# kemingy/rabitq

Measured on AMD Instinct MI355X. Metric: queries/sec at recall@10>=0.95, 100Mx128; HBM GB/s on popcount scan, higher is better.
Workload: dtype exact integer dot (fp6 MFMA, v_dot8_u32_u4) + f32

## Files before the change

include/rabitq_hip.h:

```cpp
#ifndef RABITQ_HIP_H
#define RABITQ_HIP_H

#include <stddef.h>
#include <stdint.h>

#ifdef __cplusplus
extern "C" {
#endif

typedef int32_t rq_status;
enum {
    RQ_OK = 0,
    RQ_ERR_INVALID = -1,
    RQ_ERR_DIM_MISMATCH = -2,
    RQ_ERR_IO = -3,
    RQ_ERR_HIP = -4,
    RQ_ERR_NO_DEVICE = -5,
    RQ_ERR_UNSUPPORTED = -6,
    RQ_ERR_EMPTY = -7,
    RQ_ERR_OOM = -8
};

typedef struct rq_index rq_index;

// ... 28 lines not shown

rq_status rq_build(const float *base, uint64_t n, uint32_t d, const float *centroids, uint32_t k,
                   const float *orthogonal, uint64_t seed, rq_index **out);
rq_status rq_build_device(const float *d_base, uint64_t n, uint32_t d, const float *d_centroids,
                          uint32_t k, const float *orthogonal_host, uint64_t seed, rq_index **out);
rq_status rq_build_from_path(const char *base_fvecs, const char *centroid_fvecs,
                             const float *orthogonal, uint64_t seed, rq_index **out);
rq_status rq_build_metric(const float *base, uint64_t n, uint32_t d, const float *centroids, uint32_t k,
                          const float *orthogonal, uint64_t seed, uint32_t metric, rq_index **out);
rq_status rq_build_device_metric(const float *d_base, uint64_t n, uint32_t d, const float *d_centroids,
                                 uint32_t k, const float *orthogonal_host, uint64_t seed, uint32_t metric, rq_index **out);
rq_status rq_build_from_path_metric(const char *base_fvecs, const char *centroid_fvecs,
                                    const float *orthogonal, uint64_t seed, uint32_t metric, rq_index **out);

typedef struct rq_builder rq_builder;
typedef struct {
    uint32_t struct_size;
    float ms_rotate, ms_assign, ms_quantize;
    uint64_t rows_assigned;
    uint64_t rows_in_hbm, rows_in_host_memory;
    uint64_t rows_exact_redo;
} rq_build_stats_t;
rq_status rq_builder_create(uint64_t n, uint32_t d, const float *d_centroids, uint32_t k, const float *orthogonal_host,
                            uint64_t seed, uint64_t max_device_base_bytes, rq_builder **out);
rq_status rq_builder_create_metric(uint64_t n, uint32_t d, const float *d_centroids, uint32_t k, const float *orthogonal_host,
                                   uint64_t seed, uint64_t max_device_base_bytes, uint32_t metric, rq_builder **out);
rq_status rq_builder_assign_chunk(rq_builder *b, const float *d_rows, uint64_t i0, uint64_t m);
rq_status rq_builder_order(rq_builder *b);
rq_status rq_builder_place_chunk(rq_builder *b, const float *d_rows, uint64_t i0, uint64_t m);
rq_status rq_builder_finish(rq_builder *b, rq_index **out);
void rq_builder_free(rq_builder *b);
rq_status rq_builder_stats(const rq_builder *b, rq_build_stats_t *out);

rq_status rq_kmeans_device(const float *d_base, uint64_t n, uint32_t d, uint32_t k, uint32_t iters,
                           uint32_t points_per_centroid, uint64_t seed, float *d_centroids_out);

rq_status rq_load_dir(const char *dir, rq_index **out);
rq_status rq_dump_dir(const rq_index *idx, const char *dir);
rq_status rq_load_json(const char *path, rq_index **out);
rq_status rq_dump_json(const rq_index *idx, const char *path);
void rq_free(rq_index *idx);

rq_status rq_from_arrays(uint32_t dim, uint64_t n, uint32_t k, const float *base,
                         const float *orthogonal, const float *centroids, const uint32_t *offsets,
                         const uint32_t *map_ids, const uint64_t *codes, const rq_factor_t *factors,
                         rq_index **out);
rq_status rq_from_arrays_metric(uint32_t dim, uint64_t n, uint32_t k, const float *base,
                                const float *orthogonal, const float *centroids, const uint32_t *offsets,
                                const uint32_t *map_ids, const uint64_t *codes, const rq_factor_t *factors,
                                uint32_t metric, rq_index **out);

rq_status rq_info(const rq_index *idx, rq_info_t *out);
enum { RQ_ARR_BASE = 0, RQ_ARR_ORTHOGONAL, RQ_ARR_CENTROIDS, RQ_ARR_OFFSETS, RQ_ARR_MAP_IDS,
       RQ_ARR_CODES, RQ_ARR_FACTORS };
rq_status rq_get_array(const rq_index *idx, int which, void *dst, uint64_t dst_bytes);
rq_status rq_get_device_ptr(const rq_index *idx, int which, const void **out_ptr, uint64_t *out_bytes);

rq_status rq_query(const rq_index *idx, const float *query, uint32_t len, uint32_t probe,
                   uint32_t topk, int heuristic_rank, float *out_dist, uint32_t *out_id,
                   uint32_t *out_n);
rq_status rq_query_batch(const rq_index *idx, const float *queries, uint32_t nq, uint32_t len,
                         uint32_t probe, uint32_t topk, int heuristic_rank, float *out_dist,
                         uint32_t *out_id, uint32_t *out_n);
rq_status rq_query_batch_device(const rq_index *idx, const float *d_queries, uint32_t nq,
                                uint32_t len, uint32_t probe, uint32_t topk, int heuristic_rank,
                                float *d_out_dist, uint32_t *d_out_id, uint32_t *d_out_n);
typedef struct rq_ticket rq_ticket;
rq_status rq_query_batch_device_begin(const rq_index *idx, const float *d_queries, uint32_t nq,
                                      uint32_t len, uint32_t probe, uint32_t topk, int heuristic_rank,
                                      float *d_out_dist, uint32_t *d_out_id, uint32_t *d_out_n,
                                      rq_ticket **out_ticket);
rq_status rq_query_batch_device_end(rq_ticket *ticket);

typedef struct rq_filter rq_filter;
rq_status rq_filter_create(const rq_index *idx, const uint32_t *allow_bits, uint64_t nbits, int bits_on_device,
                           rq_filter **out);
rq_status rq_filter_rows(const rq_filter *f, uint64_t *out_admitted);
void rq_filter_free(rq_filter *f);
rq_status rq_query_batch_filtered(const rq_index *idx, const rq_filter *filter, const float *queries, uint32_t nq,
                                  uint32_t len, uint32_t probe, uint32_t topk, int heuristic_rank, float *out_dist,
                                  uint32_t *out_id, uint32_t *out_n);
rq_status rq_query_batch_device_filtered(const rq_index *idx, const rq_filter *filter, const float *d_queries,
                                         uint32_t nq, uint32_t len, uint32_t probe, uint32_t topk, int heuristic_rank,
                                         float *d_out_dist, uint32_t *d_out_id, uint32_t *d_out_n);

typedef struct rq_range_result rq_range_result;
rq_status rq_range_search_device(const rq_index *idx, const rq_filter *filter, const float *d_queries, uint32_t nq,
                                 uint32_t len, uint32_t probe, const float *d_radius, rq_range_result **out);
rq_status rq_range_search(const rq_index *idx, const rq_filter *filter, const float *queries, uint32_t nq, uint32_t len,
                          uint32_t probe, const float *radius, rq_range_result **out);
rq_status rq_range_result_info(const rq_range_result *r, uint32_t *out_nq, uint64_t *out_total);
rq_status rq_range_result_device_ptrs(const rq_range_result *r, const uint64_t **d_lims, const float **d_dist,
                                      const uint32_t **d_id);
rq_status rq_range_result_copy(const rq_range_result *r, uint64_t *lims, float *dist, uint32_t *id);
void rq_range_result_free(rq_range_result *r);

typedef struct {
    uint32_t struct_size;
    uint32_t reserved0;
    float ms_keys, ms_assign, ms_alloc, ms_merge, ms_gather, ms_derive, ms_free, ms_total;
    uint64_t rows_before, rows_after;
    uint64_t gather_bytes;
} rq_mutate_stats_t;
rq_status rq_add(rq_index *idx, const float *rows, uint64_t m, uint32_t d, const uint32_t *ids, int rows_on_device,
                 uint32_t *out_first_id);
rq_status rq_remove(rq_index *idx, const uint32_t *id_bits, uint64_t nbits, int bits_on_device, uint64_t *out_removed);
rq_status rq_last_mutate_stats(rq_mutate_stats_t *out);
// ... 16 lines not shown
rq_status rq_partition_lists(const rq_index *idx, uint32_t world, uint32_t *out_owner, uint64_t *out_load);
rq_status rq_shard_index(const rq_index *idx, const uint32_t *owner, uint32_t rank, rq_index **out);
rq_status rq_query_batch_sharded_device(const rq_index *shard, void *nccl_comm, uint32_t world, uint32_t id_offset,
                                        const float *d_queries, uint32_t nq, uint32_t len, uint32_t probe, uint32_t topk,
                                        int heuristic_rank, float *d_out_dist, uint32_t *d_out_id, uint32_t *d_out_n);
typedef struct {
    uint32_t struct_size;
    uint32_t reserved;
    int (*all_gather)(const void *send, void *recv, size_t send_count, int dtype, void *comm, void *hip_stream);
    int (*all_reduce)(const void *send, void *recv, size_t count, int dtype, int op, void *comm, void *hip_stream);
    int (*comm_user_rank)(void *comm, int *rank);
} rq_collectives_t;
rq_status rq_set_collectives(const rq_collectives_t *collectives);

rq_status rq_metrics(rq_metrics_t *out);
rq_status rq_metrics_reset(void);

rq_status rq_rotate(const float *x, uint64_t n, uint32_t dim, const float *orthogonal, int use_mfma,
                    float *out);
rq_status rq_rotate_device(const rq_index *idx, const float *d_x, uint64_t n, float *d_out, float *out_ms);
rq_status rq_quantize_pack(const float *x_rot, uint64_t n, uint32_t dim, const float *centroids_rot,
                           uint32_t k, uint32_t *out_label, float *out_dist, uint64_t *out_codes,
                           rq_factor_t *out_factors);
rq_status rq_coarse_rank(const rq_index *idx, const float *queries, uint32_t nq, uint32_t len,
                         uint32_t probe, float *out_y, uint32_t *out_cluster, float *out_dist);
rq_status rq_query_prep(const rq_index *idx, const float *y, uint32_t nq, const uint32_t *cluster,
                        float *out_lower, float *out_delta, uint32_t *out_sum, uint64_t *out_planes);
rq_status rq_scan(const rq_index *idx, uint32_t cluster, float y_c_distance_square,
                  const uint64_t *planes, float lower_bound, float scalar_sum, float delta,
                  float *out_rough);
rq_status rq_rerank(const rq_index *idx, const float *query_padded, const uint32_t *pos, uint32_t m,
                    float *out_accurate);

typedef struct {
    uint32_t struct_size;
    uint32_t coarse_fallback_rows;
    float ms_rotate, ms_coarse, ms_select, ms_prep, ms_group, ms_scan, ms_rerank, ms_sort, ms_replay,
        ms_total;
    uint64_t scan_bytes;
    uint64_t scan_candidates;
    uint64_t rerank_candidates;
    uint32_t scan_launches;
    uint32_t retries;
    float ms_scan_matrix;
    uint32_t matrix_launches;
    uint64_t matrix_pairs;
    uint64_t matrix_subtile_steps, matrix_exact_steps;
    uint64_t rerank_shadow_rejects;
    float ms_early;
    uint32_t small_batch_passes;
    uint64_t survivor_workspace_bytes;
    uint32_t segmented_passes;
    uint32_t matrix_additive_launches;
} rq_profile_t;
rq_status rq_set_profiling(int level);
rq_status rq_set_option(const char *name, int value);
rq_status rq_last_profile(rq_profile_t *out);

#ifdef __cplusplus
}
#endif
#endif
```

rabitq_amd/_lib.py:

```python
from __future__ import annotations

import ctypes as C
import os
import subprocess

_HERE = os.path.dirname(os.path.abspath(__file__))
SO_PATH = os.environ.get("RABITQ_HIP_SO") or os.path.join(_HERE, "librabitq_hip.so")
CSRC = os.path.join(_HERE, "csrc")

RQ_OK = 0
RQ_ERR_EMPTY = -7
STATUS_NAMES = {0: "RQ_OK", -1: "RQ_ERR_INVALID", -2: "RQ_ERR_DIM_MISMATCH", -3: "RQ_ERR_IO", -4: "RQ_ERR_HIP",
                -5: "RQ_ERR_NO_DEVICE", -6: "RQ_ERR_UNSUPPORTED", -7: "RQ_ERR_EMPTY", -8: "RQ_ERR_OOM"}

EXPORTS = [
    "rq_version", "rq_abi_version", "rq_last_error", "rq_init", "rq_normalize", "rq_normalize_device", "rq_build", "rq_build_device", "rq_build_from_path",
    "rq_build_metric", "rq_build_device_metric", "rq_build_from_path_metric", "rq_builder_create_metric", "rq_from_arrays_metric", "rq_kmeans_device", "rq_builder_create", "rq_builder_assign_chunk", "rq_builder_order", "rq_builder_place_chunk", "rq_builder_finish", "rq_builder_free", "rq_builder_stats", "rq_load_dir",
    "rq_dump_dir", "rq_load_json", "rq_dump_json", "rq_free", "rq_from_arrays", "rq_info", "rq_get_array", "rq_get_device_ptr", "rq_query",
    "rq_query_batch", "rq_query_batch_device", "rq_query_batch_device_begin", "rq_query_batch_device_end", "rq_filter_create", "rq_filter_rows", "rq_filter_free", "rq_query_batch_filtered", "rq_query_batch_device_filtered", "rq_range_search", "rq_range_search_device", "rq_range_result_info", "rq_range_result_device_ptrs", "rq_range_result_copy", "rq_range_result_free", "rq_add", "rq_remove", "rq_last_mutate_stats", "rq_coarse_topk_device", "rq_merge_smallest_u64_device", "rq_query_batch_device_probed", "rq_query_batch_device_seeded", "rq_partition_lists", "rq_shard_index", "rq_query_batch_sharded_device", "rq_set_collectives", "rq_metrics", "rq_metrics_reset", "rq_rotate", "rq_rotate_device",
    "rq_quantize_pack",
    "rq_coarse_rank", "rq_query_prep", "rq_scan", "rq_rerank", "rq_set_profiling", "rq_set_option", "rq_last_profile",
]


class RabitqError(RuntimeError):
    def __init__(self, status, message):
        super().__init__(f"{STATUS_NAMES.get(status, status)}: {message}")
        self.status = status


METRIC_L2, METRIC_COSINE = 0, 1
METRICS = {"l2": METRIC_L2, "cosine": METRIC_COSINE}


def metric_id(metric) -> int:
    if isinstance(metric, str):
        if metric.lower() not in METRICS:
            raise ValueError(f"metric must be one of {sorted(METRICS)}, not {metric!r}")
        return METRICS[metric.lower()]
    return int(metric)


ABI_VERSION = 4


class _Sized(C.Structure):

    def __init__(self, *a, **kw):
        super().__init__(*a, **kw)
        self.struct_size = C.sizeof(type(self))


class Info(_Sized):
    _fields_ = [("struct_size", C.c_uint32), ("dim", C.c_uint32), ("k", C.c_uint32), ("max_list_len", C.c_uint32),
                ("n", C.c_uint64), ("n_hbm", C.c_uint64), ("split_rows", C.c_uint32), ("metric", C.c_uint32)]


class MetricsT(C.Structure):
    _fields_ = [("rough", C.c_uint64), ("precise", C.c_uint64), ("query", C.c_uint64), ("miss", C.c_uint64)]


class BuildStatsT(_Sized):
    _fields_ = [("struct_size", C.c_uint32), ("ms_rotate", C.c_float), ("ms_assign", C.c_float), ("ms_quantize", C.c_float),
                ("rows_assigned", C.c_uint64), ("rows_in_hbm", C.c_uint64), ("rows_in_host_memory", C.c_uint64),
                ("rows_exact_redo", C.c_uint64)]


class ProfileT(_Sized):
    _fields_ = [("struct_size", C.c_uint32), ("coarse_fallback_rows", C.c_uint32)] + [(n, C.c_float) for n in ("ms_rotate", "ms_coarse", "ms_select", "ms_prep", "ms_group", "ms_scan",
                                         "ms_rerank", "ms_sort", "ms_replay", "ms_total")] + [
        ("scan_bytes", C.c_uint64), ("scan_candidates", C.c_uint64), ("rerank_candidates", C.c_uint64),
        ("scan_launches", C.c_uint32), ("retries", C.c_uint32),
        ("ms_scan_matrix", C.c_float), ("matrix_launches", C.c_uint32), ("matrix_pairs", C.c_uint64),
        ("matrix_subtile_steps", C.c_uint64), ("matrix_exact_steps", C.c_uint64),
        ("rerank_shadow_rejects", C.c_uint64), ("ms_early", C.c_float), ("small_batch_passes", C.c_uint32),
        ("survivor_workspace_bytes", C.c_uint64), ("segmented_passes", C.c_uint32), ("matrix_additive_launches", C.c_uint32)]


class MutateStatsT(_Sized):
    _fields_ = [("struct_size", C.c_uint32), ("reserved0", C.c_uint32)] + [(n, C.c_float) for n in (
        "ms_keys", "ms_assign", "ms_alloc", "ms_merge", "ms_gather", "ms_derive", "ms_free", "ms_total")] + [
        ("rows_before", C.c_uint64), ("rows_after", C.c_uint64), ("gather_bytes", C.c_uint64)]


def build(force: bool = False) -> str:
    cmd = ["make", "-C", CSRC] + (["-B"] if force else [])
    subprocess.check_call(cmd, stdout=subprocess.DEVNULL)
    return SO_PATH


_lib = None


def lib():
    global _lib
    if _lib is not None:
        return _lib
    if not os.path.exists(SO_PATH):
        raise RabitqError(-5, f"{SO_PATH} not built (run `make -C rabitq_amd/csrc`); there is no CPU fallback")
    import importlib.util
    import sys
    if (not os.environ.get("RABITQ_NO_TORCH_PRELOAD") and "torch" not in sys.modules
            and importlib.util.find_spec("torch") is not None):
        try:
            import torch
        except Exception:
            pass
    L = C.CDLL(SO_PATH)
    vp, f32p, u32p, u64p = C.c_void_p, C.c_void_p, C.c_void_p, C.c_void_p
    u32, u64, i32, flt = C.c_uint32, C.c_uint64, C.c_int32, C.c_float
    pp = C.POINTER(C.c_void_p)
    sig = {
        "rq_version": (C.c_char_p, []),
        "rq_abi_version": (C.c_uint32, []),
        "rq_last_error": (C.c_char_p, []),
        "rq_init": (i32, [C.c_int]),
        "rq_build": (i32, [f32p, u64, u32, f32p, u32, f32p, u64, pp]),
        "rq_build_device": (i32, [f32p, u64, u32, f32p, u32, f32p, u64, pp]),
        "rq_build_from_path": (i32, [C.c_char_p, C.c_char_p, f32p, u64, pp]),
        "rq_normalize": (i32, [f32p, u64, u32, f32p]),
        "rq_normalize_device": (i32, [f32p, u64, u32, f32p]),
        "rq_build_metric": (i32, [f32p, u64, u32, f32p, u32, f32p, u64, u32, pp]),
        "rq_build_device_metric": (i32, [f32p, u64, u32, f32p, u32, f32p, u64, u32, pp]),
        "rq_build_from_path_metric": (i32, [C.c_char_p, C.c_char_p, f32p, u64, u32, pp]),
        "rq_builder_create_metric": (i32, [u64, u32, f32p, u32, f32p, u64, u64, u32, pp]),
        "rq_from_arrays_metric": (i32, [u32, u64, u32, f32p, f32p, f32p, u32p, u32p, u64p, vp, u32, pp]),
        "rq_kmeans_device": (i32, [f32p, u64, u32, u32, u32, u32, u64, f32p]),
        "rq_builder_create": (i32, [u64, u32, f32p, u32, f32p, u64, u64, pp]),
        "rq_builder_assign_chunk": (i32, [vp, f32p, u64, u64]),
# ... 69 lines not shown
```

rabitq_amd/csrc/host_build.h:

```cpp
#pragma once
#define RQ_SHADOW_MIN_ROWS 1ull
static std::atomic<int> g_rerank_shadow{2};
static rq_status derive_shadow_rows(rq_index *idx);
static rq_status finish_index(rq_index *idx) {
    idx->W = idx->dim / 64;
    RQC(idx->cent_t.alloc((size_t)idx->dim * idx->k));
    RQC(ensure_kernel_attributes());
    if (idx->k)
        transpose_kernel<<<dim3(ceil_div(idx->dim, 32), ceil_div(idx->k, 32)), dim3(32, 8)>>>(
            idx->centroids.p, idx->cent_t.p, idx->k, idx->dim);
    DevBuf<uint32_t> mx;
    RQC(mx.alloc(2));
    const uint32_t mx_init[2] = {0u, 0xFFFFFFFFu};
    HIPC(hipMemcpy(mx.p, mx_init, 8, hipMemcpyHostToDevice));
    if (idx->k) max_list_len_kernel<<<ceil_div(idx->k, 256), 256>>>(idx->offsets.p, idx->k, mx.p);
    uint32_t mx_out[2];
    HIPC(hipMemcpy(mx_out, mx.p, 8, hipMemcpyDeviceToHost));
    idx->max_list_len = mx_out[0];
    idx->min_list_len = idx->k ? mx_out[1] : 0;
    {
        DevBuf<uint32_t> st4;
        RQC(st4.alloc(4));
        HIPC(hipMemset(st4.p, 0, 16));
        if (idx->n)
            factor_stats_kernel<<<(uint32_t)std::min<uint64_t>(ceil_div(idx->n, 256), 4096), 256>>>(idx->factors.p, idx->n, st4.p);
        HIPC(hipMemcpy(&idx->fstats, st4.p, 16, hipMemcpyDeviceToHost));
    }
    idx->cent_norm_max = INFINITY;
    if (idx->k) {
        const uint64_t cells = (uint64_t)idx->k * idx->dim;
        DevBuf<uint32_t> mxb;
        RQC(mxb.alloc(1));
        HIPC(hipMemset(mxb.p, 0, 4));
        RQC(idx->cent_bf.alloc(cells));
        RQC(idx->cent_sqnorm.alloc(idx->k));
        to_bf16_kernel<<<ceil_div(cells, 2048), 256>>>(idx->centroids.p, cells, idx->cent_bf.p);
        row_sqnorm_kernel<<<ceil_div(idx->k, 256), 256>>>(idx->centroids.p, idx->k, idx->dim, idx->cent_sqnorm.p, mxb.p);
        float m2 = 0.0f;
        HIPC(hipMemcpy(&m2, mxb.p, 4, hipMemcpyDeviceToHost));
        idx->cent_norm_max = std::isfinite(m2) && m2 < 1.0e30f ? std::sqrt(m2) * 1.000001f : INFINITY;
    }
    if (idx->k) {
        RQC(idx->list_uref.alloc(idx->k));
        list_uref_kernel<<<idx->k, 256>>>(idx->factors.p, idx->offsets.p, idx->list_uref.p);
    }
    HIPC(hipDeviceSynchronize());
    HIPC(hipGetLastError());
    RQC(derive_shadow_rows(idx));
    idx->h_offsets.resize((size_t)idx->k + 1);
    HIPC(hipMemcpy(idx->h_offsets.data(), idx->offsets.p, ((size_t)idx->k + 1) * 4, hipMemcpyDeviceToHost));
    idx->nonempty_lists = 0;
    for (uint32_t c = 0; c < idx->k; ++c) idx->nonempty_lists += idx->h_offsets[c + 1] > idx->h_offsets[c] ? 1u : 0u;
    {
        size_t free_b = 0, total_b = 0;
        HIPC(hipMemGetInfo(&free_b, &total_b));
        idx->pass_budget = std::min<uint64_t>(std::max<uint64_t>(free_b / 3, 4ull << 30), 96ull << 30);
    }
    return RQ_OK;
}

static rq_status derive_shadow_rows(rq_index *idx) {
    idx->base_h.release();
    idx->base_q8.release();
    idx->list_q8.release();
    int kind = g_rerank_shadow.load();
    if (kind == 2 && idx->dim > 4096) kind = 1;
    if (!kind || idx->base_host != nullptr || idx->split_rows || idx->n < RQ_SHADOW_MIN_ROWS) return RQ_OK;
    const uint64_t total = idx->n * idx->dim, bytes = total * (kind == 2 ? 1 : 2);
    size_t free_b = 0, total_b = 0;
    HIPC(hipMemGetInfo(&free_b, &total_b));
    if (free_b < bytes + (48ull << 30) && bytes > (1ull << 30)) return RQ_OK;
    if (kind == 2) {
        if (idx->base_q8.alloc(total) != RQ_OK || idx->list_q8.alloc(std::max<uint32_t>(idx->k, 1)) != RQ_OK) {
            (void)hipGetLastError();
            idx->base_q8.release();
            idx->list_q8.release();
            return RQ_OK;
        }
        std::vector<uint32_t> off((size_t)idx->k + 1);
        HIPC(hipMemcpy(off.data(), idx->offsets.p, off.size() * 4, hipMemcpyDeviceToHost));
        uint32_t longest = 0;
        for (uint32_t c = 0; c < idx->k; ++c) longest = std::max(longest, off[c + 1] - off[c]);
        q8_range_kernel<<<idx->k, 256>>>(idx->base.p, idx->offsets.p, idx->dim, idx->list_q8.p);
        if (longest)
            for (uint32_t c0 = 0; c0 < idx->k; c0 += 32768)
                q8_encode_kernel<<<dim3(ceil_div(longest, 256u), std::min(32768u, idx->k - c0)), 256>>>(
                    idx->base.p, idx->offsets.p + c0, idx->dim, idx->list_q8.p + c0, idx->base_q8.p);
        HIPC(hipDeviceSynchronize());
        HIPC(hipGetLastError());
        return RQ_OK;
    }
    if (idx->base_h.alloc(total) != RQ_OK) {
        (void)hipGetLastError();
        return RQ_OK;
    }
    half_rows_kernel<<<(uint32_t)std::min<uint64_t>(ceil_div(total, 2048), 1u << 20), 256>>>(idx->base.p, total, idx->base_h.p);
    HIPC(hipDeviceSynchronize());
    HIPC(hipGetLastError());
    return RQ_OK;
}

static void gen_orthogonal(uint32_t dim, uint64_t seed, std::vector<float> &out) {
    std::mt19937_64 rng(seed);
    std::normal_distribution<double> nd(0.0, 1.0);
    const size_t D = dim;
    std::vector<double> A(D * D), Q(D * D, 0.0), v(D);
    for (auto &a : A) a = nd(rng);
    std::vector<std::vector<double>> vs;
    vs.reserve(D);
    for (size_t j = 0; j < D; ++j) {
        double norm = 0;
        for (size_t i = j; i < D; ++i) norm += A[i * D + j] * A[i * D + j];
        norm = std::sqrt(norm);
        std::vector<double> h(D, 0.0);
        double alpha = A[j * D + j] > 0 ? -norm : norm;
        for (size_t i = j; i < D; ++i) h[i] = A[i * D + j];
        h[j] -= alpha;
        double hn = 0;
        for (size_t i = j; i < D; ++i) hn += h[i] * h[i];
        if (hn > 0) {
            for (size_t c = j; c < D; ++c) {
                double dot = 0;
                for (size_t i = j; i < D; ++i) dot += h[i] * A[i * D + c];
                dot = 2 * dot / hn;
                for (size_t i = j; i < D; ++i) A[i * D + c] -= dot * h[i];
            }
        }
        vs.push_back(std::move(h));
    }
    for (size_t i = 0; i < D; ++i) Q[i * D + i] = 1.0;
    for (size_t jj = D; jj-- > 0;) {
        const auto &h = vs[jj];
        double hn = 0;
        for (size_t i = jj; i < D; ++i) hn += h[i] * h[i];
        if (hn == 0) continue;
        for (size_t c = 0; c < D; ++c) {
            double dot = 0;
            for (size_t i = jj; i < D; ++i) dot += h[i] * Q[i * D + c];
            dot = 2 * dot / hn;
            for (size_t i = jj; i < D; ++i) Q[i * D + c] -= dot * h[i];
// ... 670 lines not shown
```

rabitq_amd/csrc/host_mutate.h:

```cpp
#pragma once

static thread_local rq_mutate_stats_t g_mutate_stats;
struct PhaseClock {
    std::chrono::steady_clock::time_point t = std::chrono::steady_clock::now();
    float lap() {
        const auto now = std::chrono::steady_clock::now();
        const float ms = std::chrono::duration<float, std::milli>(now - t).count();
        t = now;
        return ms;
    }
};

static rq_status ensure_row_keys(rq_index *idx) {
    if (idx->row_key_valid) return RQ_OK;
    PhaseClock clk;
    const uint64_t n = idx->n;
    const uint32_t dim = idx->dim;
    DevBuf<uint32_t> rk;
    RQC(rk.alloc(n));
    if (n) {
        const uint64_t chunk = std::min<uint64_t>(n, std::max<uint64_t>(64, (256ull << 20) / ((uint64_t)dim * 4)));
        DevBuf<float> xrot;
        RQC(xrot.alloc(chunk * dim));
        for (uint64_t r0 = 0; r0 < n; r0 += chunk) {
// ... 104 lines not shown
    RQC(nx->base.alloc(n * dim));
    RQC(nx->codes.alloc(n * W));
    RQC(nx->factors.alloc(n));
    RQC(nx->map_ids.alloc(n));
    RQC(nx->row_key.alloc(n));
    DevBuf<uint32_t> src_of_dst, empty_off;
    DevBuf<unsigned int> holes;
    RQC(src_of_dst.alloc(n));
    RQC(holes.alloc(1));
    HIPC(hipMemset(holes.p, 0, 4));
    HIPC(hipMemset(src_of_dst.p, 0xFF, n * 4));
    HIPC(hipMemcpy(nx->P.p, idx->P.p, (size_t)dim * dim * 4, hipMemcpyDeviceToDevice));
    HIPC(hipMemcpy(nx->centroids.p, idx->centroids.p, (size_t)k * dim * 4, hipMemcpyDeviceToDevice));
    HIPC(hipMemcpy(nx->offsets.p, h_out.data(), ((size_t)k + 1) * 4, hipMemcpyHostToDevice));
    const uint32_t *new_off = nullptr;
    if (nr) {
        new_off = nr->off.p;
    } else {
        RQC(empty_off.alloc((size_t)k + 1));
        HIPC(hipMemset(empty_off.p, 0, ((size_t)k + 1) * 4));
        new_off = empty_off.p;
    }
    HIPC(hipDeviceSynchronize());
    st.ms_alloc = clk.lap();
    const unsigned long long *nkeys = nr ? nr->keys.p : nullptr;
    const uint32_t *nids = nr && nr->ids.p ? nr->ids.p : nullptr, *nsrc = nr && nr->src.p ? nr->src.p : nullptr;
    const uint32_t id0 = nr ? nr->id0 : 0u;
    if (k)
        mutate_merge_kernel<<<k, 256>>>(idx->offsets.p, idx->row_key.p, idx->map_ids.p, drop_bits, new_off, nkeys, nids, id0,
                                        nx->offsets.p, (uint32_t)n_old, src_of_dst.p);
    HIPC(hipDeviceSynchronize());
    st.ms_merge = clk.lap();
    if (n)
        mutate_gather_kernel<<<(uint32_t)std::min<uint64_t>(ceil_div(n, 4), 1u << 20), 256>>>(
            src_of_dst.p, n, (uint32_t)n_old, nr ? (uint32_t)nr->m : 0u, dim, W, idx->base.p, idx->codes.p, idx->factors.p, idx->map_ids.p, idx->row_key.p,
            nkeys, nids, id0, nsrc, nr ? nr->rows : nullptr, nr ? nr->d : dim, nr ? nr->b->codes_tmp.p : nullptr,
            nr ? nr->b->factors_tmp.p : nullptr, nx->base.p, nx->codes.p, nx->factors.p, nx->map_ids.p, nx->row_key.p, holes.p);
    HIPC(hipDeviceSynchronize());
    HIPC(hipGetLastError());
    st.ms_gather = clk.lap();
    st.gather_bytes = 2 * n * ((uint64_t)dim * 4 + (uint64_t)W * 8 + 16 + 4 + 4) + n * 4;
    unsigned int h_holes = 0;
    HIPC(hipMemcpy(&h_holes, holes.p, 4, hipMemcpyDeviceToHost));
    if (h_holes)
        return fail(RQ_ERR_HIP, "internal: the merge left " + std::to_string(h_holes) + " rows of the new layout unset");
    src_of_dst.release();
    if (nr) nr->b.reset();
    RQC(finish_index(nx.get()));
    nx->row_key_valid = true;
    st.ms_derive = clk.lap();

    swap_buf(idx->base, nx->base), swap_buf(idx->P, nx->P), swap_buf(idx->centroids, nx->centroids), swap_buf(idx->cent_t, nx->cent_t);
    swap_buf(idx->base_h, nx->base_h), swap_buf(idx->base_q8, nx->base_q8), swap_buf(idx->list_q8, nx->list_q8);
    swap_buf(idx->offsets, nx->offsets), swap_buf(idx->map_ids, nx->map_ids), swap_buf(idx->codes, nx->codes);
    swap_buf(idx->factors, nx->factors), swap_buf(idx->list_uref, nx->list_uref), swap_buf(idx->cent_bf, nx->cent_bf);
    swap_buf(idx->cent_sqnorm, nx->cent_sqnorm), swap_buf(idx->row_key, nx->row_key);
    idx->n = nx->n, idx->n_dev = nx->n_dev, idx->max_list_len = nx->max_list_len, idx->min_list_len = nx->min_list_len;
    idx->cent_norm_max = nx->cent_norm_max, idx->nonempty_lists = nx->nonempty_lists, idx->fstats = nx->fstats;
    idx->pass_budget = nx->pass_budget;
    idx->h_offsets.swap(nx->h_offsets);
    idx->row_key_valid = true;
    {
        std::lock_guard<std::mutex> g(idx->tt_mu);
        idx->tile_tables.clear();
    }
    {
        std::lock_guard<std::mutex> g(idx->ws_mu);
        idx->ws_pool.clear();
    }
    ++idx->generation;
    nx.reset();
    HIPC(hipDeviceSynchronize());
    st.ms_free = clk.lap();
    if (!idx->base_q8.p && !idx->base_h.p) (void)derive_shadow_rows(idx);
    size_t free_b = 0, total_b = 0;
    if (hipMemGetInfo(&free_b, &total_b) == hipSuccess)
        idx->pass_budget = std::min<uint64_t>(std::max<uint64_t>(free_b / 3, 4ull << 30), 96ull << 30);
    (void)hipGetLastError();
    st.ms_derive += clk.lap();
    return RQ_OK;
}

static rq_status scan_ids(const rq_index *idx, const uint32_t *sorted, uint64_t m, uint64_t *top, uint64_t *hits) {
    DevBuf<unsigned long long> out;
    RQC(out.alloc(2));
    HIPC(hipMemset(out.p, 0, 16));
    if (idx->n)
        id_scan_kernel<<<(uint32_t)std::min<uint64_t>(ceil_div(idx->n, 256), 4096), 256>>>(idx->map_ids.p, idx->n, sorted, (uint32_t)m, out.p);
    unsigned long long h[2];
    HIPC(hipMemcpy(h, out.p, 16, hipMemcpyDeviceToHost));
    *top = h[0], *hits = h[1];
    return RQ_OK;
}

static void mutate_stats_begin(const rq_index *idx) {
    g_mutate_stats = rq_mutate_stats_t{};
    g_mutate_stats.struct_size = sizeof(rq_mutate_stats_t);
    g_mutate_stats.rows_before = g_mutate_stats.rows_after = idx ? idx->n : 0;
}

static rq_status index_add(rq_index *idx, const float *rows, uint64_t m, uint32_t d, const uint32_t *ids, int rows_on_device,
                           uint32_t *out_first_id) {
    RQC(ensure_device());
    RQC(ensure_kernel_attributes());
    mutate_stats_begin(idx);
    RQC(mutate_refusals(idx));
// ... 100 lines not shown
```

rabitq_amd/csrc/host_plan.h:

```cpp
#pragma once
struct QueryParams {
    uint32_t nq, len, probe, topk;
    bool heuristic;
    uint32_t cap, hcap;
    const float *thr_init = nullptr;
    bool seg_final = false;
    bool ext_lists = false;
    const rq_filter *filter = nullptr;
    bool range = false;
};

#define RQ_DEFAULT_CAP 4096u
#define RQ_MAX_CAP_HINT 32768u
#define RQ_MAX_NQ_PER_PASS 65536u
#define RQ_MAX_PROBE 16384u

#define RQ_PREP_SHAPES(X) X(128, 16, 2, 16, 2) X(64, 16, 1, 16, 4) X(256, 32, 2, 8, 2) X(512, 32, 4, 8, 1) X(768, 32, 6, 8, 1) X(1024, 32, 8, 8, 1)

struct StagePlan {
    uint32_t s_lo, s_hi;
    uint64_t span, est_pairs;
    bool matrix;
    bool cluster_major;
    bool ranked;
    bool additive;
    bool arena_stage;
    bool placed;
    bool want_table;
    uint32_t slot_hi, stage_pairs;
    uint32_t dense_cells;
    uint32_t tile, tiles_per_group;
};

struct PassPlan {
    uint32_t nprobe, npairs;
    uint32_t dbg;
    bool small;
    uint32_t sb_nstages, sb_lo[RQ_SB_MAX_STAGES], sb_hi[RQ_SB_MAX_STAGES], sb_final_lo;
    bool sb_whole, sb_fill_final;
    bool will_list;
    bool placed;
    bool fin_additive;
    bool write_qn, write_q6;
    uint32_t qn_slots;
    uint32_t prep_lp, prep_r, prep_ppb, prep_pp;
    uint32_t mid_blocks;
    uint32_t nstages;
    StagePlan st[RQ_MAX_STAGES];
};

static void plan_stages(const rq_index *idx, uint32_t nq, uint32_t nprobe, uint64_t first_hi, uint64_t growth, uint64_t settle_cap, PassPlan &pl) {
    pl.nstages = 0;
    const uint64_t total_max = std::min<uint64_t>((uint64_t)nprobe * idx->max_list_len, idx->n);
    uint64_t lo = 0, hi = first_hi;
    const uint64_t avg = std::max<uint64_t>(1, idx->n / std::max<uint32_t>(idx->nonempty_lists, 1));
    uint64_t settle = std::min(settle_cap, std::max<uint64_t>(avg, std::min<uint64_t>(idx->max_list_len, 16 * avg)));
    if (rq_large_batch(nq)) settle = std::max<uint64_t>(1, settle * (uint64_t)g_stage_settle_pct.load() / 100);
    while (lo < total_max) {
        const bool last = hi >= total_max || lo >= settle || pl.nstages + 1 == RQ_MAX_STAGES;
        pl.st[pl.nstages++] = StagePlan{(uint32_t)lo, last ? 0xFFFFFFFFu : (uint32_t)hi};
        if (last) break;
        lo = hi;
        hi = std::min<uint64_t>(hi * growth, 0xFFFFFFF0ull);
        if (lo < 2 * avg && 2 * hi > 2 * avg) hi = 2 * avg;
        if (lo < settle && hi > settle) hi = settle;
    }
}

static void plan_pass(const rq_index *idx, const QueryParams &qp, bool has_row_map, bool ext_lists, PassPlan &pl) {
    const uint32_t dim = idx->dim, k = idx->k, W = idx->W;
    const uint32_t nq = qp.nq, nprobe = std::min(qp.probe, k), topk = qp.topk;
    const uint32_t npairs = nq * nprobe;
    const rq_filter *filt = qp.filter;
    const bool large = rq_large_batch(nq), fused = scan_is_fused(W);
    pl = PassPlan{};
    pl.nprobe = nprobe, pl.npairs = npairs;
    const uint32_t min_len = filt ? 0u : idx->min_list_len;
    const int impl = g_scan_impl.load();
    pl.dbg = (uint32_t)g_scan_dbg.load();
    const int gate_opt = g_scan_gate.load(), rank_opt = g_group_rank.load(), tt_opt = g_scan_tile_table.load(), gopt = g_stage_growth.load();
    const bool dense_opt = g_dense_dir.load() != 0, additive_loose = idx->additive_loose.load() != 0;
    const uint64_t settle_pct = (uint64_t)g_stage_settle_pct.load();
    const uint64_t avg_len = std::max<uint64_t>(1, idx->n / std::max<uint32_t>(idx->nonempty_lists, 1));
    const uint64_t total_max = std::min<uint64_t>((uint64_t)nprobe * idx->max_list_len, idx->n);
    const bool one_stage = qp.range || (qp.thr_init != nullptr && !has_row_map);

    const bool sb_w = W == 1 || W == 2 || W == 4 || W == 8 || W == 12 || W == 16;
    pl.small = g_small_batch.load() == 0 && nq <= RQ_SB_MAX_NQ && !ext_lists && !has_row_map && !qp.thr_init && !filt && sb_w &&
               k <= RQ_SB_MAX_K && nprobe <= 64 && topk <= RQ_SB_MAX_TOPK && qp.cap <= 4 * RQ_DEFAULT_CAP;
    if (pl.small) {
        plan_stages(idx, nq, nprobe, 16ull * std::max<uint32_t>(topk, 1), gopt >= 2 ? (uint64_t)gopt : 8, (uint64_t)std::max(1, g_sb_span.load()), pl);
        if (pl.nstages > RQ_SB_MAX_STAGES) pl.small = false;
    }
    if (pl.small) {
        const bool whole = pl.sb_whole = pl.nstages == 0 || (total_max - pl.st[pl.nstages - 1].s_lo) * (uint64_t)(dim / 8 + 16) <= (1ull << 20);
        pl.sb_nstages = whole ? pl.nstages : pl.nstages - 1;
        for (uint32_t i = 0; i < pl.sb_nstages; ++i) pl.sb_lo[i] = pl.st[i].s_lo, pl.sb_hi[i] = pl.st[i].s_hi;
        const StagePlan fin = whole ? StagePlan{} : pl.st[pl.nstages - 1];
        pl.sb_fill_final = !whole && !(npairs >= k / 2 && npairs > 64);
        pl.sb_final_lo = fin.s_lo;
        pl.nstages = 0;
        if (!whole) pl.st[pl.nstages++] = fin;
    } else if (one_stage) {
        pl.nstages = 1;
        pl.st[0] = StagePlan{0u, 0xFFFFFFFFu};
    } else {
        const uint64_t growth = gopt >= 2 ? (uint64_t)gopt : (nq >= 32768 ? 8 : 16);
        plan_stages(idx, nq, nprobe, (uint64_t)std::max<uint32_t>(topk, 1) * (large ? growth : 1), growth, ~0ull, pl);
    }

    for (uint32_t i = 0; i < pl.nstages; ++i) {
        StagePlan &s = pl.st[i];
        s.span = (uint64_t)std::min<uint64_t>(s.s_hi, (uint64_t)nprobe * idx->max_list_len) - s.s_lo;
        s.est_pairs = (uint64_t)nq * std::min<uint64_t>(nprobe, s.span / avg_len + 2);
        s.matrix = scan_has_mfma(W) && impl != 1 &&
                   (impl == 2 || (s.est_pairs >= 8ull * k && (s.s_lo >= avg_len * settle_pct / 100 || one_stage)));
        s.cluster_major = s.matrix || (s.est_pairs >= k / (pl.small ? 2u : (uint32_t)g_cluster_major_div.load()) && s.est_pairs > 64);
        s.arena_stage = qp.seg_final && s.span > qp.cap && fused && large;
        s.additive = s.matrix && !s.arena_stage && !filt && scan_has_additive(W) && idx->list_uref.p != nullptr && gate_opt != 1 &&
                     (gate_opt == 2 || !additive_loose);
        s.slot_hi = nprobe;
        if (s.cluster_major && min_len > 0 && !ext_lists && s.s_hi != 0xFFFFFFFFu)
            s.slot_hi = (uint32_t)std::min<uint64_t>(nprobe, (uint64_t)(s.s_hi - 1) / min_len + 1);
        s.stage_pairs = nq * s.slot_hi;
        s.ranked = s.cluster_major && k <= 32768 &&
                   (rank_opt == 2 || (rank_opt == 1 && s.stage_pairs >= 16 * RQ_RANK_ITEMS && s.stage_pairs / RQ_RANK_ITEMS >= k / 256));
        s.tile = s.matrix ? scan_mfma_tile(W, s.arena_stage, s.additive) : scan_tile(W);
        s.tiles_per_group = ceil_div(std::min<uint64_t>(idx->max_list_len, s.s_hi), s.tile);
        const uint64_t grid_blocks = (uint64_t)k * s.tiles_per_group, real_tiles = idx->n / s.tile + k;
        s.want_table = s.cluster_major && fused && s.s_hi >= idx->max_list_len && (tt_opt == 2 || (tt_opt == 1 && grid_blocks > 4 * real_tiles));
        if (large && !s.matrix && fused && dense_opt && s.s_hi != 0xFFFFFFFFu && !(qp.seg_final && s.span > qp.cap)) {
            const uint64_t cells = (uint64_t)((s.s_hi - 1) >> 6) - (s.s_lo >> 6) + 2ull * s.slot_hi + 2;
// ... 40 lines not shown
```

rabitq_amd/csrc/host_query.h:

```cpp
#pragma once
static rq_status ws_prepare(const rq_index *idx, Workspace &ws, const QueryParams &qp) {
    const uint32_t nprobe = std::min(qp.probe, idx->k);
    const uint64_t nq = qp.nq, npairs = nq * nprobe;
    if (!ws.stream) HIPC(hipStreamCreateWithFlags(&ws.stream, hipStreamNonBlocking));
    if (!ws.h_totals) HIPC(hipHostMalloc((void **)&ws.h_totals, 16 * sizeof(unsigned long long)));
    RQC(ws.qpad.ensure(nq * idx->dim));
    RQC(ws.y.ensure(nq * idx->dim));
    if (!qp.ext_lists) RQC(ws.dist.ensure(nq * idx->k));
    RQC(ws.probe_dist.ensure(npairs));
    RQC(ws.probe_cluster.ensure(npairs));
    RQC(ws.scal.ensure(npairs));
    if (!scan_is_fused(idx->W)) RQC(ws.planes.ensure(npairs * 4 * idx->W));
    RQC(ws.qnib.ensure(npairs * 8 * idx->W));
    RQC(ws.qf6.ensure(npairs * 12 * idx->W));
    RQC(ws.rough_cnt.ensure(nq));
    RQC(ws.totals.ensure(16));
    RQC(ws.stat.ensure(256));
    RQC(ws.recs.ensure((npairs + 32ull * idx->k + 32) * (12ull * idx->W + 2 + RQ_REC_TAIL)));
    RQC(ws.grp_cnt.ensure(idx->k + 4));
    RQC(ws.grp_start.ensure(idx->k + 1));
    RQC(ws.q_hist.ensure(idx->k + 2));
    RQC(ws.q_start.ensure(idx->k + 2));
    RQC(ws.q_order.ensure(nq));
    RQC(ws.thr.ensure(nq));
    RQC(ws.surv.ensure(nq * qp.cap));
    RQC(ws.runs.ensure(nq * qp.cap));
    ws.use_runs_tmp = qp.cap > RQ_DEFAULT_CAP || qp.seg_final || hints_of(idx, qp.filter).big_dirs.load() > 0;
    if (ws.use_runs_tmp) RQC(ws.runs_tmp.ensure(nq * qp.cap));
    RQC(ws.surv_cnt.ensure(nq));
    RQC(ws.heap_len.ensure(nq));
    RQC(ws.heap_key.ensure(nq * qp.topk));
    RQC(ws.heap_id.ensure(nq * qp.topk));
    RQC(ws.precise.ensure(nq));
    RQC(ws.need.ensure(nq));
    RQC(ws.ovf.ensure(nq));
    RQC(ws.q_cap.ensure(nq));
    RQC(ws.q_base.ensure(nq));
    RQC(ws.nsurv.ensure(nq));
    RQC(ws.nshadow.ensure(nq));
    RQC(ws.recent.ensure(nq));
    RQC(ws.win_count.ensure(nq));
    RQC(ws.arr_len.ensure(nq));
    RQC(ws.row_map.ensure(nq));
    RQC(ws.big_list.ensure(nq + 3));
    if (qp.heuristic) RQC(ws.arr.ensure(nq * qp.hcap));
    return RQ_OK;
}

struct PassResult {
    uint64_t rough = 0, precise = 0, overflowed = 0, max_need = 0;
};

static rq_status finish_pass(const rq_index *idx, Workspace &ws, PassResult *res, rq_profile_t *prof_acc) {
    Prof &pf = ws.prof;
    const uint32_t nq = ws.pend.nq, dim = idx->dim;
    HIPC(hipStreamSynchronize(ws.stream));
    HIPC(hipGetLastError());
    res->rough = ws.h_totals[0];
    res->precise = ws.h_totals[1];
    res->overflowed = ws.h_totals[2];
    res->max_need = ws.h_totals[4];
    if (rq_large_batch(nq) && !ws.pend.range) hints_of(idx, ws.pend.filter).big_dirs.store((uint32_t)ws.h_totals[7]);
    if (ws.pend.additive && !ws.pend.range && ws.h_totals[8] >= 4096 && ws.h_totals[9] * 32 > ws.h_totals[8])
        const_cast<rq_index *>(idx)->additive_loose.store(1);
    if (prof_acc) prof_acc->matrix_subtile_steps += ws.h_totals[8], prof_acc->matrix_exact_steps += ws.h_totals[9];
    if (prof_acc) prof_acc->coarse_fallback_rows += (uint32_t)std::min<unsigned long long>(ws.h_totals[10], 0xFFFFFFFFull);
    if (pf.on && prof_acc) {
        float ms[PF_N] = {0};
        pf.collect(ms);
        prof_acc->ms_rotate += ms[PF_ROTATE], prof_acc->ms_coarse += ms[PF_COARSE];
        prof_acc->ms_select += ms[PF_SELECT], prof_acc->ms_prep += ms[PF_PREP], prof_acc->ms_group += ms[PF_GROUP];
        prof_acc->ms_scan += ms[PF_SCAN] + ms[PF_SCAN_MATRIX], prof_acc->ms_scan_matrix += ms[PF_SCAN_MATRIX];
        prof_acc->ms_rerank += ms[PF_RERANK], prof_acc->ms_sort += ms[PF_SORT];
        if (ws.pend.n_matrix_ranges) {
            std::vector<unsigned long long> len(nq);
            HIPC(hipMemcpy(len.data(), ws.pend.filter ? ws.stream_len.p : ws.rough_cnt.p, (size_t)nq * 8, hipMemcpyDeviceToHost));
            for (uint32_t i = 0; i < ws.pend.n_matrix_ranges; ++i) {
                const StreamRange r = ws.pend.matrix_ranges[i];
                for (uint32_t b = 0; b < nq; ++b)
                    prof_acc->matrix_pairs += std::min<unsigned long long>(len[b], r.s_hi) - std::min<unsigned long long>(len[b], r.s_lo);
            }
        }
        prof_acc->ms_replay += ms[PF_REPLAY], prof_acc->ms_total += ms[PF_TOTAL], prof_acc->ms_early += ms[PF_EARLY];
    }
    if (prof_acc) {
        const uint64_t slots = std::max<uint64_t>((uint64_t)nq * ws.pend.cap, ws.pend.seg_slots);
        prof_acc->survivor_workspace_bytes = std::max<uint64_t>(prof_acc->survivor_workspace_bytes,
            ws.pend.seg_slots ? (ws.surv.count + ws.runs.count + ws.runs_tmp.count + ws.arena_recs.count + ws.arena_runs.count) * 16ull
                              : slots * (ws.use_runs_tmp ? 48ull : 32ull));
        prof_acc->segmented_passes += ws.pend.seg_slots ? 1u : 0u;
        prof_acc->scan_candidates += res->rough;
        prof_acc->scan_bytes += res->rough * (uint64_t)(dim / 8 + 16);
        prof_acc->rerank_candidates += ws.h_totals[3];
        prof_acc->rerank_shadow_rejects += ws.h_totals[5];
        if (g_scan_dbg.load() & 256) {
            unsigned long long ht[12];
            HIPC(hipMemcpy(ht, ws.stat.p + 128, sizeof ht, hipMemcpyDeviceToHost));
            if (ht[3])
                fprintf(stderr, "[rabitq_hip] scan_mfma exact path (wave 0 of every block): %.0f cycles per block inside it (of which flushes %.0f), "
                        "%.1f flagged registers, %.1f with survivors and %.2f flushes per block\n", (double)ht[5] / ht[3], (double)ht[6] / ht[3],
                        (double)ht[9] / ht[3], (double)ht[7] / ht[3], (double)ht[8] / ht[3]);
            if (ht[3])
                fprintf(stderr, "[rabitq_hip] scan_mfma timing: %llu blocks, %.1f tiles/block; per block cycles: start-up %.0f, "
                        "tile-loop waits %.0f, tile bodies %.0f (per tile: wait %.0f, body %.0f)\n", ht[3], (double)ht[4] / ht[3],
                        (double)ht[0] / ht[3], (double)ht[1] / ht[3], (double)ht[2] / ht[3], (double)ht[1] / std::max(1ull, ht[4]),
                        (double)ht[2] / std::max(1ull, ht[4]));
        }
        if ((g_scan_dbg.load() & 4096) && nq <= RQ_SB_MAX_NQ) {
            unsigned long long hs[32];
            HIPC(hipMemcpy(hs, ws.stat.p, sizeof hs, hipMemcpyDeviceToHost));
            std::string line = "[rabitq_hip] sb_query_kernel phases (us since entry):";
            for (unsigned long long i = 1; i < std::min<unsigned long long>(hs[0], 30); ++i) line += " " + std::to_string((hs[1 + i] - hs[1]) / 100.0).substr(0, 6);
            fprintf(stderr, "%s\n", line.c_str());
        }
    }
    return RQ_OK;
}

struct StageRun {
    const StagePlan &s;
    uint32_t no;
    ScanArgs a{};
    ScanPtrs sp{};
    QSeg seg{};
    bool runs_in_tmp = false;
};
struct Pass {
    const rq_index *idx;
    Workspace &ws;
    const QueryParams &qp;
    const PassPlan &pl;
    Prof &pf;
    hipStream_t st;
    const uint32_t dim, k, W, nq, topk, nprobe, npairs;
    const float *d_q;
    const uint32_t *d_row_map, *ext_cluster;
    const float *ext_dist;
    float *d_out_dist;
    uint32_t *d_out_id, *d_out_n;
    rq_profile_t *prof_acc;
    const float *qpad;
    const uint32_t *probe_cluster;
    const float *probe_dist;
    ReplayState rs;
    const uint32_t *rerank_order = nullptr;
    uint32_t nlive = 0;
    bool sb_results_done = false;
// ... 342 lines not shown
            if (s.dense_cells) {
                pf.begin(PF_SORT);
                clear_dir_kernel<<<ceil_div((uint64_t)qp.nq * s.dense_cells, 256), 256, 0, st>>>(ws.runs.p, qp.nq, r.seg, s.dense_cells);
                pf.end();
            }
            stage_launch_scan(r);
        }
        if (s.matrix) pend.matrix_stages++;
        if (prof_acc && s.additive) prof_acc->matrix_additive_launches++;
        if (prof_acc) prof_acc->scan_launches++;
        if (prof_acc && s.matrix) {
            prof_acc->matrix_launches++;
            pend.matrix_ranges[pend.n_matrix_ranges++] = {s.s_lo, s.s_hi};
        }
        return RQ_OK;
    }

    void stage_finish_small(StageRun &r) {
        const QSeg &seg = r.seg;
        pf.begin(PF_RERANK);
        const uint32_t fin_threads = nq <= 16 ? 1024u : 256u;
        uint32_t flags = qp.cap > RQ_DEFAULT_CAP && nprobe <= 1024 ? 1u : 0u;
        if (flags) {
            sort_runs_kernel<<<nq, 64, 0, st>>>(ws.runs.p, ws.surv_cnt.p, seg, ws.big_list.p, ws.big_list.p + nq, RQ_SORT_LDS_RECS, nullptr);
            sort_runs_mid_kernel<<<std::min(nq, 256u), 256, RQ_SORT_MID_LDS_WORDS * 8, st>>>(ws.runs.p, ws.use_runs_tmp ? ws.runs_tmp.p : nullptr, ws.surv_cnt.p,
                                                                                          seg, ws.big_list.p, ws.big_list.p + nq, nprobe, 0u,
                                                                                          RQ_SORT_MID_LDS_WORDS);
        }
        if (pl.small && !qp.heuristic) {
            if (nq <= 32) {
                accurate_kernel<<<dim3(std::max(1u, std::min(16u, 256u / nq)), nq), 256, (size_t)dim * sizeof(float), st>>>(
                    ws.surv.p, ws.surv_cnt.p, seg, idx->view(), qpad, dim, nullptr, probe_cluster, nprobe);
                flags |= 2u;
            }
            auto finish = topk < 64 ? sb_finish_kernel<true> : sb_finish_kernel<false>;
            finish<<<nq, fin_threads, (size_t)dim * sizeof(float) + (2 * RQ_SBF_RUNS + RQ_SBF_RECS) * 16, st>>>(
                ws.surv.p, ws.runs.p, ws.surv_cnt.p, seg, idx->view(), qpad, dim, topk, rs, probe_cluster, nprobe, flags,
                idx->map_ids.p, d_out_dist, d_out_id, d_out_n, ws.rough_cnt.p, ws.totals.p);
            sb_results_done = true;
        } else {
            auto finish = qp.heuristic ? stage_finish_kernel<true> : stage_finish_kernel<false>;
            finish<<<nq, fin_threads, (size_t)dim * sizeof(float), st>>>(ws.surv.p, ws.runs.p, ws.surv_cnt.p, seg, idx->view(), qpad, dim, topk, rs,
                                                                         probe_cluster, nprobe, flags);
        }
        pf.end();
    }

    void stage_finish_large(StageRun &r) {
        const uint32_t dense_cells = r.s.dense_cells;
        const QSeg &seg = r.seg;
        pf.begin(PF_RERANK);
        const uint32_t gx = std::max(1u, std::min(16u, 4096u / std::max(nq, 1u)));
        const bool prefilter = (r.no > 0 || qp.thr_init) && !(pl.dbg & 512);
        if (idx->base_q8.p && prefilter)
            accurate_filtered8_kernel<<<dim3(gx, nq), 256, (size_t)dim * sizeof(float) + (nprobe <= RQ_ACC8_LDS_PROBES ? (size_t)nprobe * 16 : 0), st>>>(
                ws.surv.p, ws.surv_cnt.p, seg, idx->base.p, idx->base_q8.p, idx->list_q8.p, qpad, dim, rerank_order, ws.thr.p,
                probe_cluster, nprobe, ws.nshadow.p, k);
        else if (idx->base_h.p && prefilter)
            accurate_filtered_kernel<<<dim3(gx, nq), 256, (size_t)dim * sizeof(float), st>>>(
                ws.surv.p, ws.surv_cnt.p, seg, idx->base.p, idx->base_h.p, qpad, dim, rerank_order, ws.thr.p,
                ws.nshadow.p);
        else if (idx->split_rows && prefilter)
            accurate_split_kernel<<<dim3(gx, nq), 256, (size_t)dim * sizeof(float) + (nprobe <= RQ_ACC8_LDS_PROBES ? (size_t)nprobe * 16 : 0), st>>>(
                ws.surv.p, ws.surv_cnt.p, seg, idx->view(), qpad, dim, rerank_order, ws.thr.p, probe_cluster, nprobe, ws.nshadow.p);
        else
            accurate_kernel<<<dim3(gx, nq), 256, (size_t)dim * sizeof(float), st>>>(ws.surv.p, ws.surv_cnt.p, seg, idx->view(), qpad, dim,
                                                                                    rerank_order, probe_cluster, nprobe);
        if (qp.range)
            range_count_kernel<<<ceil_div(nq, 4), 256, 0, st>>>(ws.surv.p, ws.surv_cnt.p, qp.cap, ws.thr.p, nq, ws.range_hits.p, ws.need.p,
                                                                ws.ovf.p, ws.precise.p, ws.nsurv.p);
        pf.end();
        if (qp.range) return;
        if (!dense_cells) {
            pf.begin(PF_SORT);
            sort_runs_kernel<<<nq, 64, 0, st>>>(ws.runs.p, ws.surv_cnt.p, seg, ws.big_list.p, ws.big_list.p + nq, 512u,
                                                r.runs_in_tmp ? ws.runs_tmp.p : nullptr);
            sort_runs_mid_kernel<<<pl.mid_blocks, 256, RQ_SORT_MID_LDS_WORDS * 8, st>>>(ws.runs.p, (ws.use_runs_tmp || r.runs_in_tmp) ? ws.runs_tmp.p : nullptr,
                                                                                       ws.surv_cnt.p, seg, ws.big_list.p, ws.big_list.p + nq, nprobe,
                                                                                       r.runs_in_tmp ? 1u : 0u, RQ_SORT_MID_LDS_WORDS);
            pf.end();
        }
        pf.begin(PF_REPLAY);
        if (qp.heuristic)
            replay_kernel<true><<<nq, 64, 16, st>>>(ws.surv.p, ws.runs.p, ws.surv_cnt.p, seg, topk, rs, dense_cells);
        else if (topk < 64)
            replay_kernel<false, true><<<nq, 64, 16, st>>>(ws.surv.p, ws.runs.p, ws.surv_cnt.p, seg, topk, rs, dense_cells);
        else
            replay_kernel<false><<<nq, 64, (size_t)topk * 8, st>>>(ws.surv.p, ws.runs.p, ws.surv_cnt.p, seg, topk, rs, dense_cells);
        pf.end();
    }

    rq_status results(size_t total_span) {
        pf.begin(PF_REPLAY);
        if (!sb_results_done) {
            if (qp.heuristic && !qp.range) {
                sort_survivors_kernel<<<nq, 256, 0, st>>>(ws.arr.p, ws.arr_len.p, qp.hcap);
                finalize_heuristic_kernel<<<ceil_div((uint64_t)nq * topk, 256), 256, 0, st>>>(rs, nq, topk, d_row_map, idx->map_ids.p,
                                                                                               d_out_dist, d_out_id, d_out_n);
            } else if (!qp.range) {
                finalize_heap_kernel<<<ceil_div((uint64_t)nq * topk, 256), 256, 0, st>>>(rs, nq, topk, d_row_map, idx->map_ids.p, d_out_dist,
                                                                                          d_out_id, d_out_n);
            }
            metrics_sum_kernel<<<std::min(256u, ceil_div(nq, 256)), 256, 0, st>>>(
                ws.rough_cnt.p, ws.precise.p, ws.need.p, qp.heuristic ? ws.arr_len.p : nullptr, ws.nsurv.p, ws.nshadow.p, nq, ws.ovf.p, qp.hcap,
                ws.totals.p);
        }
        pf.end();
        if (pf.on) (void)hipEventRecord(pf.spans[total_span].b, st);
        HIPC(hipMemcpyAsync(ws.h_totals, ws.totals.p, 7 * sizeof(unsigned long long), hipMemcpyDeviceToHost, st));
        ws.h_totals[7] = 0, ws.h_totals[8] = 0, ws.h_totals[9] = 0, ws.h_totals[10] = 0;
        if (pend.prefiltered) HIPC(hipMemcpyAsync(ws.h_totals + 10, ws.totals.p + 12, 8, hipMemcpyDeviceToHost, st));
        if (pend.matrix_stages) {
            stat_fold_kernel<<<1, 64, 0, st>>>(ws.stat.p, ws.stat.p + 200);
            HIPC(hipMemcpyAsync(ws.h_totals + 8, ws.stat.p + 200, 16, hipMemcpyDeviceToHost, st));
        }
        if (rq_large_batch(nq))
            HIPC(hipMemcpyAsync(ws.h_totals + 7, ws.big_list.p + nq + 2, 4, hipMemcpyDeviceToHost, st));
        ws.pend = pend;
        return RQ_OK;
    }
};

static rq_status run_pass(const rq_index *idx, Workspace &ws, const float *d_q, const QueryParams &qp,
                          const uint32_t *d_row_map, float *d_out_dist, uint32_t *d_out_id, uint32_t *d_out_n,
                          PassResult *res, rq_profile_t *prof_acc, const uint32_t *ext_cluster = nullptr,
                          const float *ext_dist = nullptr, bool defer = false) {
    PassPlan pl;
    plan_pass(idx, qp, d_row_map != nullptr, ext_cluster != nullptr, pl);
    Pass c{idx, ws, qp, pl, ws.prof, ws.stream, idx->dim, idx->k, idx->W, qp.nq, qp.topk, pl.nprobe, pl.npairs, d_q, d_row_map, ext_cluster, ext_dist,
           d_out_dist, d_out_id, d_out_n, prof_acc, d_q, ws.probe_cluster.p, ws.probe_dist.p};
    c.rs.thr = ws.thr.p, c.rs.heap_len = ws.heap_len.p, c.rs.heap_key = ws.heap_key.p, c.rs.heap_id = ws.heap_id.p;
    c.rs.precise = ws.precise.p, c.rs.need = ws.need.p, c.rs.nsurv = ws.nsurv.p, c.rs.nshadow = ws.nshadow.p, c.rs.recent_max = ws.recent.p, c.rs.win_count = ws.win_count.p;
    c.rs.arr_len = ws.arr_len.p, c.rs.arr = ws.arr.p, c.rs.hcap = qp.hcap, c.rs.ovf = ws.ovf.p;
    c.pend.nq = qp.nq, c.pend.cap = qp.cap, c.pend.filter = qp.filter, c.pend.range = qp.range;
    Prof &pf = ws.prof;
    pf.reset(g_profiling.load(), ws.stream);
    pf.begin(PF_TOTAL);
    const size_t total_span = pf.spans.size() ? pf.spans.size() - 1 : 0;
    if (pl.small) {
        RQC(c.small_front());
    } else {
        RQC(c.rotate_coarse());
        if (pl.placed) RQC(c.place_final());
        pf.begin(PF_PREP);
        RQC(c.quantise());
        RQC(c.orders_state());
        pf.end();
    }
    for (uint32_t i = 0; i < pl.nstages; ++i) {
        StageRun r{pl.st[i], i};
        RQC(c.stage_group_fill(r));
        RQC(c.stage_scan(r));
        if (!qp.range && !rq_large_batch(qp.nq) && qp.cap <= 4 * RQ_DEFAULT_CAP) c.stage_finish_small(r);
        else c.stage_finish_large(r);
    }
    RQC(c.results(total_span));
    if (defer) return RQ_OK;
    return finish_pass(idx, ws, res, prof_acc);
}

static rq_status validate_call(const rq_index *idx, bool args_null, uint32_t len, uint32_t probe, uint32_t topk, const rq_filter *filter) {
    RQC(ensure_device());
    RQC(ensure_kernel_attributes());
    if (!idx || args_null) return fail(RQ_ERR_INVALID, "null argument");
    if (idx->dim != (len + 63) / 64 * 64)
        return fail(RQ_ERR_DIM_MISMATCH, "query length " + std::to_string(len) + " does not pad to index dim " +
                                             std::to_string(idx->dim));
    if (probe == 0 || idx->k == 0) return fail(RQ_ERR_INVALID, "probe == 0 (the reference panics at rabitq.rs:295)");
    if (topk == 0 || topk > RQ_MAX_TOPK) return fail(RQ_ERR_UNSUPPORTED, "topk must be in [1, 2048]");
    if (std::min(probe, idx->k) > RQ_MAX_PROBE) return fail(RQ_ERR_UNSUPPORTED, "probe > 16384 not supported");
    if (idx->dim > 4096) return fail(RQ_ERR_UNSUPPORTED, "dim > 4096 not supported");
    if (filter && filter->idx != idx) return fail(RQ_ERR_INVALID, "the filter was made for another index");
    if (filter && filter->generation != idx->generation)
        return fail(RQ_ERR_INVALID, "the filter was made before the index was last mutated (rq_add / rq_remove): make it again");
    return RQ_OK;
}
static rq_status validate_query(const rq_index *idx, const float *d_q, uint32_t len, uint32_t probe, uint32_t topk,
                                const float *d_out_dist, const uint32_t *d_out_id, const uint32_t *d_out_n, const rq_filter *filter = nullptr) {
    return validate_call(idx, !d_q || !d_out_dist || !d_out_id || !d_out_n, len, probe, topk, filter);
}

static uint32_t pass_capacity(const rq_index *idx, uint32_t remaining, bool seeded, bool *seg, const rq_filter *filter = nullptr) {
    const uint32_t hint = hints_of(idx, filter).cap.load();
    const int opt = g_seg_opt.load();
    *seg = !seeded && rq_large_batch(remaining) && scan_is_fused(idx->W) && (opt >= 2 || (opt == 1 && hint > RQ_DEFAULT_CAP));
// ... 309 lines not shown
```

rabitq_amd/csrc/host_shard.h:

```cpp
#pragma once
rq_status rq_partition_lists(const rq_index *idx, uint32_t world, uint32_t *out_owner, uint64_t *out_load) {
    if (!idx || !out_owner || world == 0) return fail(RQ_ERR_INVALID, "bad partition arguments");
    std::vector<uint32_t> off((size_t)idx->k + 1);
    RQC(rq_get_array(idx, RQ_ARR_OFFSETS, off.data(), off.size() * 4));
    std::vector<uint32_t> order(idx->k);
    for (uint32_t c = 0; c < idx->k; ++c) order[c] = c;
    std::stable_sort(order.begin(), order.end(),
                     [&](uint32_t a, uint32_t b) { return off[a + 1] - off[a] > off[b + 1] - off[b]; });
    typedef std::pair<uint64_t, uint32_t> LS;
    std::priority_queue<LS, std::vector<LS>, std::greater<LS>> heap;
    for (uint32_t r = 0; r < world; ++r) heap.push({0, r});
    for (uint32_t c : order) {
        LS t = heap.top();
        heap.pop();
        out_owner[c] = t.second;
        t.first += off[c + 1] - off[c];
        heap.push(t);
    }
    if (out_load) {
        for (uint32_t r = 0; r < world; ++r) out_load[r] = 0;
        for (uint32_t c = 0; c < idx->k; ++c) out_load[out_owner[c]] += off[c + 1] - off[c];
    }
    return RQ_OK;
}
// ... 37 lines not shown
}

struct RcclApi {
    int (*all_gather)(const void *, void *, size_t, int, void *, hipStream_t) = nullptr;
    int (*all_reduce)(const void *, void *, size_t, int, int, void *, hipStream_t) = nullptr;
    int (*user_rank)(void *, int *) = nullptr;
    const char *(*error_string)(int) = nullptr;
    std::string err;
};
static RcclApi g_custom_coll;
static std::atomic<bool> g_use_custom_coll{false};
static RcclApi *rccl_api() {
    if (g_use_custom_coll.load()) return &g_custom_coll;
    static RcclApi api;
    static std::once_flag once;
    std::call_once(once, [] {
        void *h = nullptr;
        const char *env = getenv("RABITQ_RCCL_LIB");
        if (env && *env) h = dlopen(env, RTLD_NOW | RTLD_GLOBAL);
        void *sym = h ? dlsym(h, "ncclAllGather") : dlsym(RTLD_DEFAULT, "ncclAllGather");
        if (!sym && !h) {
            for (const char *name : {"librccl.so.1", "librccl.so"}) {
                h = dlopen(name, RTLD_NOW | RTLD_GLOBAL);
                if (h) break;
            }
            sym = h ? dlsym(h, "ncclAllGather") : nullptr;
        }
        if (!sym) {
            api.err = "RCCL not found (ncclAllGather): set RABITQ_RCCL_LIB to the librccl.so the communicator came from";
            return;
        }
        auto find = [&](const char *name) { return h ? dlsym(h, name) : dlsym(RTLD_DEFAULT, name); };
        api.all_gather = reinterpret_cast<decltype(api.all_gather)>(sym);
        api.all_reduce = reinterpret_cast<decltype(api.all_reduce)>(find("ncclAllReduce"));
        api.user_rank = reinterpret_cast<decltype(api.user_rank)>(find("ncclCommUserRank"));
        api.error_string = reinterpret_cast<decltype(api.error_string)>(find("ncclGetErrorString"));
    });
    return &api;
}
#define RQ_NCCL_INT32 2
#define RQ_NCCL_UINT64 5
#define RQ_NCCL_FLOAT32 7
#define RQ_NCCL_MAX 2
#define RQ_NCCL_MIN 3

static void profile_add(rq_profile_t &acc, const rq_profile_t &x) {
    acc.ms_rotate += x.ms_rotate, acc.ms_coarse += x.ms_coarse, acc.ms_select += x.ms_select, acc.ms_prep += x.ms_prep;
    acc.ms_group += x.ms_group, acc.ms_scan += x.ms_scan, acc.ms_rerank += x.ms_rerank, acc.ms_sort += x.ms_sort;
    acc.ms_replay += x.ms_replay, acc.ms_total += x.ms_total, acc.scan_bytes += x.scan_bytes;
    acc.scan_candidates += x.scan_candidates, acc.rerank_candidates += x.rerank_candidates, acc.scan_launches += x.scan_launches;
    acc.retries += x.retries, acc.ms_scan_matrix += x.ms_scan_matrix, acc.matrix_launches += x.matrix_launches;
    acc.matrix_pairs += x.matrix_pairs, acc.matrix_subtile_steps += x.matrix_subtile_steps;
    acc.matrix_exact_steps += x.matrix_exact_steps, acc.rerank_shadow_rejects += x.rerank_shadow_rejects;
    acc.ms_early += x.ms_early, acc.small_batch_passes += x.small_batch_passes;
    acc.survivor_workspace_bytes = std::max(acc.survivor_workspace_bytes, x.survivor_workspace_bytes), acc.segmented_passes += x.segmented_passes;
    acc.matrix_additive_launches += x.matrix_additive_launches;
    acc.coarse_fallback_rows += x.coarse_fallback_rows;
}

__global__ void pack_probe_keys_kernel(const uint32_t *__restrict__ pc, const float *__restrict__ pd, uint64_t cells,
                                       unsigned long long *__restrict__ keys) {
    const uint64_t i = (uint64_t)blockIdx.x * blockDim.x + threadIdx.x;
    if (i < cells) keys[i] = ((unsigned long long)__builtin_bit_cast(uint32_t, pd[i]) << 32) | pc[i];
}
__global__ void unpack_probe_keys_kernel(const unsigned long long *__restrict__ keys, uint32_t nq, uint32_t npb,
                                         uint32_t *__restrict__ pc, float *__restrict__ pd, uint32_t *__restrict__ pc_a,
                                         float *__restrict__ pd_a, uint32_t *__restrict__ pc_b, float *__restrict__ pd_b) {
    const uint64_t i = (uint64_t)blockIdx.x * blockDim.x + threadIdx.x;
    if (i >= (uint64_t)nq * npb) return;
    const uint32_t b = (uint32_t)(i / npb), c = (uint32_t)(i - (uint64_t)b * npb);
    const unsigned long long key = keys[i];
    const uint32_t id = (uint32_t)key;
    const float dv = __builtin_bit_cast(float, (uint32_t)(key >> 32));
    pc[i] = id, pd[i] = dv;
    if (!pc_a) return;
    if (c == 0) pc_a[b] = id, pd_a[b] = dv;
    else pc_b[(uint64_t)b * (npb - 1) + c - 1] = id, pd_b[(uint64_t)b * (npb - 1) + c - 1] = dv;
}
__global__ void gather_status_kernel(const unsigned long long *__restrict__ gathered, uint32_t world, uint64_t rank_stride,
                                     uint64_t at, uint32_t *__restrict__ flag) {
    uint32_t bad = 0;
    for (uint32_t w = 0; w < world; ++w) bad |= gathered[(uint64_t)w * rank_stride + at] != 0ull ? (w + 1u) : 0u;
    *flag = bad;
}

static rq_status sharded_step(rq_index *mi, void *nccl_comm, uint32_t world, uint32_t id_offset, const float *d_queries,
                              uint32_t nq, uint32_t len, uint32_t probe, uint32_t topk, bool heuristic, float *d_out_dist,
                              uint32_t *d_out_id, uint32_t *d_out_n, bool shared) {
    RcclApi *api = nccl_comm ? rccl_api() : nullptr;
    if (api && (!api->all_gather || !api->all_reduce))
        return fail(RQ_ERR_UNSUPPORTED, api->err.empty() ? "ncclAllGather / ncclAllReduce not found" : api->err);
    if (api && world > 1 && !api->user_rank) return fail(RQ_ERR_UNSUPPORTED, "ncclCommUserRank not found");
    auto nccl_fail = [&](const char *what, int rc) {
        return fail(RQ_ERR_HIP, std::string(what) + ": " + (api && api->error_string ? api->error_string(rc) : "error " + std::to_string(rc)));
    };
    const uint32_t npb = std::min(probe, std::max(mi->k, 1u));
    const uint32_t width = shared ? 2 * topk : topk;
    Workspace *ws = ws_acquire(mi);
    WsLease rel(mi, ws);
    if (!ws->stream) HIPC(hipStreamCreateWithFlags(&ws->stream, hipStreamNonBlocking));
    hipStream_t st = ws->stream;
    RQC(ws->sh_flag.ensure(8));
    const uint64_t cells = (uint64_t)nq * topk, pcells = (uint64_t)nq * npb;
    const uint64_t out_stride = (uint64_t)nq * width + 1;
    int my_rank = 0;
    rq_status err = validate_query(mi, d_queries, len, probe, topk, d_out_dist, d_out_id, d_out_n);
// ... 164 lines not shown
```

rabitq_amd/csrc/host_state.h:

```cpp
#pragma once
static thread_local std::string g_err;
static rq_status fail(rq_status s, const std::string &msg) {
    g_err = msg;
    return s;
}
#define HIPC(expr)                                                                                   \
    do {                                                                                             \
        hipError_t _e = (expr);                                                                      \
        if (_e != hipSuccess)                                                                        \
            return fail(_e == hipErrorOutOfMemory ? RQ_ERR_OOM : RQ_ERR_HIP,                         \
                        std::string(#expr) + ": " + hipGetErrorString(_e));                          \
    } while (0)
#define RQC(expr)                        \
    do {                                 \
        rq_status _s = (expr);           \
        if (_s != RQ_OK) return _s;      \
    } while (0)

static rq_status ensure_device() {
    int count = 0;
    hipError_t e = hipGetDeviceCount(&count);
    if (e != hipSuccess || count == 0)
        return fail(RQ_ERR_NO_DEVICE, "no HIP device visible (librabitq_hip has no CPU fallback)");
    return RQ_OK;
// ... 111 lines not shown
    void reset(int level, hipStream_t st) {
        on = level != 0;
        light = level == 2;
        stream = st;
        spans.clear();
        used = 0;
        open = false;
        last_b = nullptr;
        failed = false;
    }
    void collect(float *ms ) {
        if (failed) return;
        for (auto &s : spans) {
            float t = 0;
            (void)hipEventElapsedTime(&t, s.a, s.b);
            ms[s.cat] += t;
        }
    }
    ~Prof() {
        for (auto e : pool) (void)hipEventDestroy(e);
    }
};

struct StreamRange {
    uint32_t s_lo, s_hi;
};
#define RQ_MAX_STAGES 40
struct PendingPass {
    uint64_t seg_slots = 0;
    uint32_t cap = 0;
    uint32_t nq = 0;
    StreamRange matrix_ranges[RQ_MAX_STAGES];
    uint32_t n_matrix_ranges = 0;
    const struct rq_filter *filter = nullptr;
    bool additive = false;
    uint32_t matrix_stages = 0;
    bool prefiltered = false;
    bool range = false;
};
struct Workspace {
    hipStream_t stream = nullptr;
    bool busy = false;
    PendingPass pend;
    DevBuf<float> qpad, y, dist, probe_dist, thr, recent;
    DevBuf<float> qnorm;
    DevBuf<float> retry_q, retry_pd, retry_pc;
    DevBuf<uint32_t> retry_rows;
    DevBuf<uint32_t> q_hist, q_start, q_order;
    DevBuf<uint32_t> live_list;
    DevBuf<uint32_t> coarse_redo;
    DevBuf<uint32_t> pair_rank, rank_base;
    DevBuf<uint32_t> img_final, pair_begin, fin_rank, fin_rank_base, fin_grp_cnt, fin_grp_start;
    DevBuf<uint32_t> probe_cluster, recs, grp_cnt, grp_start, heap_len, heap_id, precise, need,
        nsurv, nshadow, win_count, arr_len, row_map, big_list;
    DevBuf<int32_t> heap_key;
    DevBuf<PairScalars> scal;
    DevBuf<uint64_t> planes;
    DevBuf<uint32_t> qnib;
    DevBuf<uint32_t> qf6;
    DevBuf<unsigned long long> rough_cnt, totals, surv_cnt, stat;
    DevBuf<unsigned long long> stream_len;
    DevBuf<float4> grp_vref;
    DevBuf<SurvRec> surv, arr;
    DevBuf<RunRec> runs, runs_tmp;
    bool use_runs_tmp = false;
    bool arena_failed = false;
    DevBuf<float> sh_dist;
    DevBuf<uint32_t> sh_id, sh_n;
    DevBuf<unsigned long long> sh_packed, sh_gathered, sh_merged;
    DevBuf<uint32_t> range_hits;
    DevBuf<uint32_t> range_lists;
    DevBuf<unsigned long long> range_counters;
    DevBuf<uint32_t> ovf, q_cap;
    DevBuf<unsigned long long> q_base;
    DevBuf<SurvRec> arena_recs;
    DevBuf<RunRec> arena_runs;
    DevBuf<uint2> arena_places;
    DevBuf<unsigned long long> arena_cur;
    DevBuf<unsigned int> arena_fail;
    DevBuf<ScanExtra> scan_extra;
    DevBuf<uint32_t> sh_flag;
    DevBuf<uint32_t> sh_pc, sh_id_b, sh_n_b;
    DevBuf<float> sh_pd, sh_thr, sh_dist_b;
    unsigned long long *h_totals = nullptr;
    Prof prof;
    ~Workspace() {
        if (h_totals) (void)hipHostFree(h_totals);
        if (stream) (void)hipStreamDestroy(stream);
    }
};

struct rq_index {
    uint32_t dim = 0, k = 0, W = 0, max_list_len = 0;
    uint32_t min_list_len = 0;
    uint64_t n = 0;
    uint32_t metric = RQ_METRIC_L2;
    uint64_t n_dev = 0;
    float *base_host = nullptr;
    float *base_host_dev = nullptr;
    DevBuf<ListTier> list_tier;
    std::vector<ListTier> h_list_tier;
    bool split_rows = false;
    BaseView view() const { return BaseView{base.p, base_host_dev, list_tier.p, k, split_rows ? 1u : 0u}; }
    ~rq_index() {
        if (base_host) (void)hipHostFree(base_host);
    }
    DevBuf<float> base, P, centroids, cent_t;
    DevBuf<_Float16> base_h;
    DevBuf<uint8_t> base_q8;
    DevBuf<float4> list_q8;
    DevBuf<uint32_t> offsets, map_ids;
    DevBuf<uint64_t> codes;
    DevBuf<float4> factors;
    DevBuf<float4> list_uref;
    DevBuf<uint16_t> cent_bf;
    DevBuf<float> cent_sqnorm;
    float cent_norm_max = INFINITY;
    uint32_t nonempty_lists = 0;
    std::atomic<int> additive_loose{0};
    std::mutex ws_mu;
    std::vector<std::unique_ptr<Workspace>> ws_pool;
    FactorStats fstats{0, 0, 0, 0};
    std::atomic<uint32_t> cap_hint{0};
    std::atomic<uint64_t> arena_hint{0};
    std::atomic<uint32_t> big_dirs_hint{0};
    std::atomic<uint32_t> range_cap_hint{0};
    uint64_t pass_budget = 24ull << 30;
    std::vector<uint32_t> h_offsets;
    std::mutex tt_mu;
    std::map<uint32_t, std::unique_ptr<DevBuf<uint4>>> tile_tables;
    DevBuf<uint32_t> row_key;
    bool row_key_valid = false;
    bool row_order_ok = true;
    bool is_shard = false;
    uint64_t generation = 0;
    std::atomic<int> open_tickets{0};
};

struct rq_filter {
    const rq_index *idx = nullptr;
    uint64_t generation = 0;
    DevBuf<uint32_t> pos_bits;
    DevBuf<uint32_t> sub_off;
    DevBuf<ScanExtra> extra;
    uint64_t rows = 0;
    std::atomic<uint32_t> cap_hint{0};
    std::atomic<uint64_t> arena_hint{0};
    std::atomic<uint32_t> big_dirs_hint{0};
};
struct PassHints {
    std::atomic<uint32_t> &cap;
    std::atomic<uint64_t> &arena;
    std::atomic<uint32_t> &big_dirs;
};
static PassHints hints_of(const rq_index *idx, const rq_filter *f) {
    if (f) {
        rq_filter *m = const_cast<rq_filter *>(f);
        return PassHints{m->cap_hint, m->arena_hint, m->big_dirs_hint};
    }
    rq_index *m = const_cast<rq_index *>(idx);
    return PassHints{m->cap_hint, m->arena_hint, m->big_dirs_hint};
}

// ... 246 lines not shown
    const uint32_t gchunk = std::max(1u, maxb / tchunk);
    for (uint32_t t0 = 0; t0 < a.tiles_per_group; t0 += tchunk)
        for (uint32_t g0 = 0; g0 < a.ngroups; g0 += gchunk) {
            ScanArgs c = a;
            c.tile_base = t0, c.group_base = g0;
            c.tiles_per_group = std::min(tchunk, a.tiles_per_group - t0);
            c.ngroups = std::min(gchunk, a.ngroups - g0);
            launch(c, dim3(c.ngroups * c.tiles_per_group));
        }
}

#define SCAN_ARGS p.codes, p.factors, p.offsets, p.grp_start, p.recs, p.surv, p.runs, p.surv_cnt, p.tile_table, a
template <bool ARENA, bool FILT>
static void launch_scan_t(const ScanPtrs &p, const ScanArgs &args, uint32_t W, hipStream_t st) {
    launch_scan_chunks(args, [&](const ScanArgs &a, dim3 g) {
        const dim3 b(256);
#define RQ_SCAN_K(WW, CPL)                                                                        \
    do {                                                                                          \
        if constexpr (FILT) scan_kernel<WW, CPL, ARENA, true><<<g, b, 0, st>>>(SCAN_ARGS);         \
        else scan_kernel<WW, CPL, ARENA><<<g, b, 0, st>>>(SCAN_ARGS);                             \
    } while (0)
        switch (W) {
            case 1: RQ_SCAN_K(1, 2); break;
            case 2: RQ_SCAN_K(2, 2); break;
            case 3: RQ_SCAN_K(3, 2); break;
            case 4: RQ_SCAN_K(4, 2); break;
            case 6: RQ_SCAN_K(6, 2); break;
            case 8: RQ_SCAN_K(8, 2); break;
            case 12: RQ_SCAN_K(12, 1); break;
            case 16: RQ_SCAN_K(16, 1); break;
            default:
                if constexpr (!ARENA && FILT) scan_generic_filtered_kernel<<<g, b, 0, st>>>(SCAN_ARGS, W);
                else if constexpr (!ARENA) scan_generic_kernel<<<g, b, 0, st>>>(SCAN_ARGS, W);
                break;
        }
#undef RQ_SCAN_K
    });
}
static void launch_scan(const ScanPtrs &p, const ScanArgs &args, uint32_t W, hipStream_t st) {
    if (p.filtered) {
        if (p.arena) launch_scan_t<true, true>(p, args, W, st);
        else launch_scan_t<false, true>(p, args, W, st);
    } else if (p.arena) launch_scan_t<true, false>(p, args, W, st);
    else launch_scan_t<false, false>(p, args, W, st);
}
static std::atomic<int> g_scan_impl{0};
static std::atomic<int> g_scan_gate{0};
static std::atomic<int> g_stage_growth{0};
static std::atomic<int> g_large_from{256};
static bool rq_large_batch(uint32_t nq) { return nq >= (uint32_t)g_large_from.load(); }
static std::atomic<int> g_cluster_major_div{32};
static std::atomic<int> g_stage_settle_pct{100};
static std::atomic<int> g_scan_tile_table{1};
static std::atomic<int> g_prep_placement{1};
static std::atomic<int> g_group_rank{1};
static std::atomic<int> g_shared_thr{1};
static std::atomic<int> g_sb_span{2560};
static std::atomic<int> g_seg_opt{1};
static std::atomic<int> g_pass_overlap{1};
static std::atomic<int> g_small_batch{0};
static std::atomic<int> g_dense_dir{1};

static bool scan_has_mfma(uint32_t W) {
    switch (W) {
        case 1: case 2: case 3: case 4: case 6: case 8: case 12: case 16: return true;
        default: return false;
    }
}
static uint32_t scan_mfma_nt(uint32_t W, bool additive = false) { return W == 2 ? (additive ? RQ_ADD_NT2 : RQ_NT_W2) : (W == 12 ? RQ_NT_W12 : (W >= 4 ? 2 : 4)); }
static uint32_t scan_mfma_nw(uint32_t W, bool arena) { return W == 2 && !arena ? 8u : 4u; }
static uint32_t scan_mfma_tile(uint32_t W, bool arena, bool additive = false) { return 32 * scan_mfma_nw(W, arena) * scan_mfma_nt(W, additive && !arena); }
static size_t scan_mfma_ring_bytes(uint32_t W, bool arena = false) {
    (void)arena;
    const uint64_t slots = W <= 2 ? 4ull : (W >= 16 ? 5ull : 3ull);
    return slots * (32 * (12 * W + 2) + RQ_REC_TAIL * 32) * 4;
}
template <int W, int NT, bool ARENA, bool ADD = false, bool FILT = false>
static void launch_scan_mfma_t(const ScanPtrs &p, const ScanArgs &a, dim3 g, hipStream_t st) {
    scan_mfma_kernel<W, NT, ARENA, ADD, FILT><<<g, dim3(64 * scan_mfma_waves<W, ARENA>()), scan_mfma_ring_bytes(W, ARENA), st>>>(p.codes, p.factors, p.offsets, p.grp_start, p.grp_cnt,
                                                                                    p.recs, p.surv, p.runs, p.surv_cnt, p.stat, p.tile_table, p.list_uref, p.grp_vref, a);
}
static bool scan_has_additive(uint32_t W) { return W == 1 || W == 2; }
static void launch_scan_mfma_add(const ScanPtrs &p, const ScanArgs &args, uint32_t W, hipStream_t st) {
    launch_scan_chunks(args, [&](const ScanArgs &a, dim3 g) {
        switch (W) {
            case 1: launch_scan_mfma_t<1, 4, false, true>(p, a, g, st); break;
            case 2: launch_scan_mfma_t<2, RQ_ADD_NT2, false, true>(p, a, g, st); break;
            default: break;
        }
    });
}
template <bool ARENA, bool FILT = false>
static void launch_scan_mfma_a(const ScanPtrs &p, const ScanArgs &args, uint32_t W, hipStream_t st) {
    launch_scan_chunks(args, [&](const ScanArgs &a, dim3 g) {
        switch (W) {
            case 1: launch_scan_mfma_t<1, 4, ARENA, false, FILT>(p, a, g, st); break;
            case 2: launch_scan_mfma_t<2, RQ_NT_W2, ARENA, false, FILT>(p, a, g, st); break;
            case 3: launch_scan_mfma_t<3, 4, ARENA, false, FILT>(p, a, g, st); break;
            case 4: launch_scan_mfma_t<4, 2, ARENA, false, FILT>(p, a, g, st); break;
            case 6: launch_scan_mfma_t<6, 2, ARENA, false, FILT>(p, a, g, st); break;
            case 8: launch_scan_mfma_t<8, 2, ARENA, false, FILT>(p, a, g, st); break;
            case 12: launch_scan_mfma_t<12, RQ_NT_W12, ARENA, false, FILT>(p, a, g, st); break;
            case 16: launch_scan_mfma_t<16, 2, ARENA, false, FILT>(p, a, g, st); break;
            default: break;
        }
    });
// ... 111 lines not shown
```

rabitq_amd/csrc/kernels_query.h:

```cpp
#pragma once
#ifndef RQ_COLLECT_UNROLL
#define RQ_COLLECT_UNROLL 8
#endif
#include "common.h"
#include "kernels_scan_common.h"

#pragma clang fp contract(off)

__global__ void pad_rows_kernel(const float *__restrict__ in, float *__restrict__ out, uint64_t n,
                                uint32_t len, uint32_t dim) {
    uint64_t i = (uint64_t)blockIdx.x * blockDim.x + threadIdx.x;
    if (i >= n * dim) return;
    uint64_t r = i / dim;
    uint32_t c = (uint32_t)(i - r * dim);
    out[i] = c < len ? in[r * len + c] : 0.0f;
}

__global__ __launch_bounds__(256) void rotate_valu_kernel(const float *__restrict__ x,
                                                          const float *__restrict__ P,
                                                          float *__restrict__ out, uint64_t n,
                                                          uint32_t dim) {
    uint64_t r = (uint64_t)blockIdx.x * 4 + threadIdx.y;
    uint32_t j = blockIdx.y * 64 + threadIdx.x;
    if (r >= n) return;
// ... 1834 lines not shown
    __syncthreads();
    {
        const uint32_t per = (nwords + nthr - 1) / nthr, w0 = tid * per < nwords ? tid * per : nwords;
        const uint32_t w1 = w0 + per < nwords ? w0 + per : nwords;
        uint32_t sum = 0;
        for (uint32_t i = w0; i < w1; ++i) sum += (uint32_t)__popc(words[i]);
        uint32_t incl = sum;
        for (int o = 1; o < 64; o <<= 1) {
            const uint32_t up = __shfl_up(incl, o, 64);
            if ((int)lane >= o) incl += up;
        }
        __syncthreads();
        if (lane == 63) bsum[wave] = incl;
        __syncthreads();
        uint32_t run = incl - sum, all = 0;
        for (uint32_t w = 0; w < (nthr >> 6); ++w) {
            if (w < wave) run += bsum[w];
            all += bsum[w];
        }
        if (all != n) return false;
        for (uint32_t i = w0; i < w1; ++i) {
            wpre[i] = run;
            run += (uint32_t)__popc(words[i]);
        }
    }
    __syncthreads();
    for (uint32_t i = tid; i < n; i += nthr) {
        const RunRec r = src[i];
        const uint32_t cell = cellbase[r.slot] + ((r.pos - minpos[r.slot]) >> 5);
        out[wpre[cell >> 5] + (uint32_t)__popc(words[cell >> 5] & ((1u << (cell & 31u)) - 1u))] = r;
    }
    return true;
}

__global__ __launch_bounds__(256) void sort_survivors_kernel(SurvRec *__restrict__ surv,
                                                             const uint32_t *__restrict__ surv_cnt,
                                                             uint32_t cap) {
    const uint32_t b = blockIdx.x;
    uint32_t n = surv_cnt[b];
    n = n < cap ? n : cap;
    sort_segment(surv + (uint64_t)b * cap, n);
}

struct ReplayState {
    float *thr;
    uint32_t *heap_len;
    int32_t *heap_key;
    uint32_t *heap_id;
    uint32_t *precise;
    uint32_t *need;
    uint32_t *ovf;
    uint32_t *nsurv;
    uint32_t *nshadow;
    float *recent_max;
    uint32_t *win_count;
    uint32_t *arr_len;
    SurvRec *arr;
    uint32_t hcap;
};

#define RQ_MAX_TOPK 2048

template <bool HEURISTIC, bool REGHEAP = false, bool CONTIG = false>
__device__ __forceinline__ void replay_wave(const SurvRec *__restrict__ recs, const RunRec *__restrict__ dir,
                                            uint32_t nruns, uint32_t topk,
                                            uint32_t b, const ReplayState &st, int32_t *hkey, uint32_t *hid) {
    const uint32_t lane = threadIdx.x & 63;
    nruns = __builtin_amdgcn_readfirstlane(nruns);
    topk = __builtin_amdgcn_readfirstlane(topk);
    float thr = st.thr[b];
    uint32_t precise = 0;
    uint32_t hlen = 0, wcount = 0, alen = 0;
    float recent = 0.0f;
    int32_t rk = 0;
    uint32_t ri = 0;
    auto HK = [&](uint32_t idx) -> int32_t {
        if constexpr (REGHEAP) return __builtin_amdgcn_readlane(rk, (int)idx);
        else return hkey[idx];
    };
    auto HI = [&](uint32_t idx) -> uint32_t {
        if constexpr (REGHEAP) return (uint32_t)__builtin_amdgcn_readlane((int)ri, (int)idx);
        else return hid[idx];
    };
    auto SETH = [&](uint32_t idx, int32_t k, uint32_t i) {
        if constexpr (REGHEAP) {
            rk = lane == idx ? k : rk;
            ri = lane == idx ? i : ri;
        } else {
            hkey[idx] = k, hid[idx] = i;
        }
    };
    if constexpr (!HEURISTIC) {
        hlen = __builtin_amdgcn_readfirstlane(st.heap_len[b]);
        if constexpr (REGHEAP) {
            if (lane < hlen) rk = st.heap_key[(uint64_t)b * topk + lane], ri = st.heap_id[(uint64_t)b * topk + lane];
        } else {
            for (uint32_t i = lane; i < hlen; i += 64) {
                hkey[i] = st.heap_key[(uint64_t)b * topk + i];
                hid[i] = st.heap_id[(uint64_t)b * topk + i];
            }
        }
    } else {
        recent = st.recent_max[b];
        wcount = __builtin_amdgcn_readfirstlane(st.win_count[b]);
        alen = __builtin_amdgcn_readfirstlane(st.arr_len[b]);
    }
// ... 446 lines not shown
#pragma unroll
                    for (int u = 0; u < 8; ++u) {
                        if (!(u < 4 || full)) continue;
                        const float4 qa = *reinterpret_cast<const float4 *>(acc_q + c + 16 * u + 8 * hf);
                        const float4 qb = *reinterpret_cast<const float4 *>(acc_q + c + 16 * u + 8 * hf + 4);
                        const float x0 = __builtin_bit_cast(float, xv[u].x << 16), x1 = __builtin_bit_cast(float, xv[u].x & 0xFFFF0000u);
                        const float x2 = __builtin_bit_cast(float, xv[u].y << 16), x3 = __builtin_bit_cast(float, xv[u].y & 0xFFFF0000u);
                        const float x4 = __builtin_bit_cast(float, xv[u].z << 16), x5 = __builtin_bit_cast(float, xv[u].z & 0xFFFF0000u);
                        const float x6 = __builtin_bit_cast(float, xv[u].w << 16), x7 = __builtin_bit_cast(float, xv[u].w & 0xFFFF0000u);
                        const float e0 = x0 - qa.x, e1 = x1 - qa.y, e2 = x2 - qa.z, e3 = x3 - qa.w;
                        const float e4 = x4 - qb.x, e5 = x5 - qb.y, e6 = x6 - qb.z, e7 = x7 - qb.w;
                        d0 = fmaf(e0, e0, d0), d1 = fmaf(e1, e1, d1), d0 = fmaf(e2, e2, d0), d1 = fmaf(e3, e3, d1);
                        d0 = fmaf(e4, e4, d0), d1 = fmaf(e5, e5, d1), d0 = fmaf(e6, e6, d0), d1 = fmaf(e7, e7, d1);
                        n0 = fmaf(x0, x0, n0), n1 = fmaf(x1, x1, n1), n0 = fmaf(x2, x2, n0), n1 = fmaf(x3, x3, n1);
                        n0 = fmaf(x4, x4, n0), n1 = fmaf(x5, x5, n1), n0 = fmaf(x6, x6, n0), n1 = fmaf(x7, x7, n1);
                    }
                }
                float dt = d0 + d1, nx = n0 + n1;
                dt += __shfl_xor(dt, 1, 2), nx += __shfl_xor(nx, 1, 2);
                const float err = (sqrtf(nx) * up) * 3.9216e-3f + 1.0e-37f;
                const float t = sqrtf(dt * down) * down - err * up;
                if (t > 0.0f && (t * t) * (down * down) > thr) {
                    exact = false;
                    if (hf == 0) recs[i].accurate = __builtin_inff();
#ifndef RQ_EXP_COUNT_HOST
                    ++rejected;
#endif
                }
            }
        }
        if (exact && hf == 0) queue[atomicAdd(&qn, 1u)] = i;
        __syncthreads();
        const uint32_t waiting = qn;
        __syncthreads();
        if (waiting >= 128) {
            exact_of(queue[waiting - 128 + pair]);
            if (threadIdx.x == 0) qn = waiting - 128;
            __syncthreads();
        }
    }
    const uint32_t waiting = qn;
    if (pair < waiting) exact_of(queue[pair]);
    uint32_t rj = hf == 0 ? rejected : 0u;
#pragma unroll
    for (int o = 32; o >= 1; o >>= 1) rj += __shfl_xor(rj, o, 64);
    if ((threadIdx.x & 63) == 0 && rj) atomicAdd(&nshadow[b], rj);
}

__host__ __device__ __forceinline__ bool q8_row_norms(uint32_t dim) {
    const uint32_t tpr = dim / 16;
    return tpr >= 1 && tpr <= 64 && (tpr & (tpr - 1)) == 0;
}
__global__ __launch_bounds__(256) void q8_range_kernel(const float *__restrict__ base, const uint32_t *__restrict__ offsets, uint32_t dim,
                                                       float4 *__restrict__ list_q8) {
    __shared__ float smn[4], smx[4];
    __shared__ uint32_t sbad[4];
    const uint32_t c = blockIdx.x;
    const uint64_t e0 = (uint64_t)offsets[c] * dim, e1 = (uint64_t)offsets[c + 1] * dim;
    float mn = 3.402823466e+38f, mx = -3.402823466e+38f;
    uint32_t bad = 0;
    for (uint64_t e = e0 + threadIdx.x * 4ull; e < e1; e += 1024) {
        const float4 v = *reinterpret_cast<const float4 *>(base + e);
        const float ve[4] = {v.x, v.y, v.z, v.w};
#pragma unroll
        for (int i = 0; i < 4; ++i) {
            if (!(fabsf(ve[i]) < 3.0e38f)) bad = 1;
            mn = ve[i] < mn ? ve[i] : mn;
            mx = ve[i] > mx ? ve[i] : mx;
        }
    }
#pragma unroll
    for (int o = 32; o >= 1; o >>= 1) {
        const float a = __shfl_xor(mn, o, 64), b = __shfl_xor(mx, o, 64);
        mn = a < mn ? a : mn, mx = b > mx ? b : mx;
        bad |= __shfl_xor(bad, o, 64);
    }
    if ((threadIdx.x & 63) == 0) smn[threadIdx.x >> 6] = mn, smx[threadIdx.x >> 6] = mx, sbad[threadIdx.x >> 6] = bad;
    __syncthreads();
    if (threadIdx.x == 0) {
        for (int w = 1; w < 4; ++w) mn = smn[w] < mn ? smn[w] : mn, mx = smx[w] > mx ? smx[w] : mx, bad |= sbad[w];
        float lo = mn, sc = (mx - mn) * (1.0f / 255.0f);
        if (e1 == e0) lo = 0.0f, sc = 1.0f;
        if (!(sc > 0.0f)) sc = 1.0f;
        if (!(sc < 3.0e38f) || !(fabsf(lo) < 3.0e38f)) bad = 1;
        list_q8[c] = make_float4(bad ? 0.0f : lo, bad ? 1.0f : sc, bad ? __builtin_inff() : 0.0f, bad ? __builtin_inff() : 0.0f);
    }
}
__global__ __launch_bounds__(256) void q8_encode_kernel(const float *__restrict__ base, const uint32_t *__restrict__ offsets, uint32_t dim,
                                                        float4 *__restrict__ list_q8, uint8_t *__restrict__ out) {
    __shared__ float smax[4], snorm[4];
    const uint32_t c = blockIdx.y, r0 = offsets[c] + blockIdx.x * 256u, r1 = offsets[c + 1];
    if (r0 >= r1) return;
    const float4 par = list_q8[c];
    const float lo = par.x, sc = par.y, inv = 1.0f / sc;
    const uint32_t tpr = dim / 16, rows_per_pass = 256 / tpr;
    const uint32_t rr = threadIdx.x / tpr, g = threadIdx.x - rr * tpr;
    const bool row_norms = q8_row_norms(dim);
    float emax = 0.0f, nmax = 0.0f;
    for (uint32_t r = r0 + rr; r < r1 && r < r0 + 256u && rr < rows_per_pass; r += rows_per_pass) {
        float e2 = 0.0f;
        const float *x = base + (uint64_t)r * dim + 16 * g;
        uint32_t w[4];
#pragma unroll
        for (int u = 0; u < 4; ++u) {
            const float4 v = *reinterpret_cast<const float4 *>(x + 4 * u);
            const float ve[4] = {v.x, v.y, v.z, v.w};
            w[u] = 0;
#pragma unroll
            for (int i = 0; i < 4; ++i) {
                float t = rintf((ve[i] - lo) * inv);
                t = t < 0.0f ? 0.0f : (t > 255.0f ? 255.0f : t);
                const uint32_t code = (uint32_t)t;
                const float e = fabsf(ve[i] - fmaf(sc, (float)code, lo));
                emax = (e > emax || !(e < 3.0e38f)) ? (e < 3.0e38f ? e : __builtin_inff()) : emax;
                e2 = fmaf(e, e, e2);
                w[u] |= code << (8 * i);
            }
        }
        *reinterpret_cast<uint4 *>(out + (uint64_t)r * dim + 16 * g) = make_uint4(w[0], w[1], w[2], w[3]);
        if (row_norms) {
            for (uint32_t o = tpr >> 1; o >= 1; o >>= 1) e2 += __shfl_xor(e2, (int)o, 64);
            nmax = (e2 > nmax || !(e2 < 3.0e38f)) ? (e2 < 3.0e38f ? e2 : __builtin_inff()) : nmax;
        }
    }
#pragma unroll
    for (int o = 32; o >= 1; o >>= 1) {
        const float a = __shfl_xor(emax, o, 64), b = __shfl_xor(nmax, o, 64);
        emax = a > emax ? a : emax, nmax = b > nmax ? b : nmax;
    }
    if ((threadIdx.x & 63) == 0) smax[threadIdx.x >> 6] = emax, snorm[threadIdx.x >> 6] = nmax;
    __syncthreads();
    if (threadIdx.x == 0) {
        for (int w2 = 1; w2 < 4; ++w2) emax = smax[w2] > emax ? smax[w2] : emax, nmax = snorm[w2] > nmax ? snorm[w2] : nmax;
        atomicMax(reinterpret_cast<unsigned int *>(&list_q8[c].z), __builtin_bit_cast(unsigned int, emax));
        const float nrm = sqrtf(nmax) * (1.0f + (float)(dim + 8) * 6.0e-8f);
        if (row_norms) atomicMax(reinterpret_cast<unsigned int *>(&list_q8[c].w), __builtin_bit_cast(unsigned int, nrm));
    }
}

#ifndef RQ_ACC8_WAVES
#define RQ_ACC8_WAVES 4
#endif
__global__ __launch_bounds__(256, RQ_ACC8_WAVES) void accurate_filtered8_kernel(SurvRec *__restrict__ surv,
                                                                 const unsigned long long *__restrict__ surv_cnt,
                                                                 const QSeg seg, const float *__restrict__ base,
                                                                 const uint8_t *__restrict__ base_q8, const float4 *__restrict__ list_q8,
                                                                 const float *__restrict__ qpad, uint32_t dim,
                                                                 const uint32_t *__restrict__ order,
                                                                 const float *__restrict__ thr_start,
                                                                 const uint32_t *__restrict__ probe_cluster, uint32_t nprobe,
                                                                 uint32_t *__restrict__ nshadow, uint32_t nlists) {
    extern __shared__ __attribute__((aligned(16))) float acc_q[];
    __shared__ uint32_t queue[512];
    __shared__ uint32_t qn;
    const uint32_t b = order ? order[blockIdx.y] : blockIdx.y;
    const uint32_t n = (uint32_t)surv_cnt[b];
    if (n > seg.capof(b) || n == 0) return;
    SurvRec *recs = surv + seg.at(b);
    const uint32_t hf = threadIdx.x & 1, pair = threadIdx.x >> 1;
    const uint32_t i_first = blockIdx.x * 256;
    SurvRec nxt[2];
    nxt[0] = recs[i_first + pair < n ? i_first + pair : 0u], nxt[1] = recs[i_first + 128 + pair < n ? i_first + 128 + pair : 0u];
    const uint32_t *pc = probe_cluster + (uint64_t)b * nprobe;
    float4 *lpar = reinterpret_cast<float4 *>(acc_q + dim);
    const bool par_lds = nprobe <= RQ_ACC8_LDS_PROBES;
    for (uint32_t c = threadIdx.x * 4; c < dim; c += 1024)
        *reinterpret_cast<float4 *>(acc_q + c) = *reinterpret_cast<const float4 *>(qpad + (uint64_t)b * dim + c);
    if (par_lds)
        for (uint32_t sl = threadIdx.x; sl < nprobe; sl += 256)
            lpar[sl] = pc[sl] < nlists ? list_q8[pc[sl]] : make_float4(0.0f, 1.0f, __builtin_inff(), __builtin_inff());
    if (threadIdx.x == 0) qn = 0;
    __syncthreads();
    const float thr = thr_start[b];
    const bool test = thr > 1e-30f && thr < 3.0e38f;
    const float eps = (float)(dim / 4 + 64) * 5.9604645e-8f, down = 1.0f - eps, up = 1.0f + eps;
    const float sqd = sqrtf((float)dim) * 1.001f;
    const bool rown = q8_row_norms(dim);
    const uint32_t ngrp = dim / 16;
    uint32_t rejected = 0;
    for (uint32_t i0 = i_first; i0 < n; i0 += gridDim.x * 256) {
        uint32_t iv[2] = {i0 + pair, i0 + 128 + pair};
        bool exact[2] = {iv[0] < n, iv[1] < n};
        const SurvRec cur[2] = {nxt[0], nxt[1]};
        {
            const uint32_t j0 = i0 + gridDim.x * 256 + pair, j1 = j0 + 128;
            nxt[0] = recs[j0 < n ? j0 : 0u], nxt[1] = recs[j1 < n ? j1 : 0u];
        }
        if (test) {
            float4 par[2];
            const uint8_t *x[2];
#pragma unroll
            for (int v = 0; v < 2; ++v) {
                par[v] = par_lds ? lpar[cur[v].slot] : list_q8[pc[cur[v].slot]];
                x[v] = base_q8 + (uint64_t)cur[v].pos * dim;
            }
            float d0[2] = {0.0f, 0.0f}, d1[2] = {0.0f, 0.0f};
            for (uint32_t g0 = hf; g0 < ngrp; g0 += 8) {
                uint4 cv[2][4];
#pragma unroll
                for (int v = 0; v < 2; ++v)
#pragma unroll
                    for (int u = 0; u < 4; ++u)
                        if (g0 + 2 * u < ngrp) cv[v][u] = *reinterpret_cast<const uint4 *>(x[v] + 16 * (g0 + 2 * u));
#pragma unroll
                for (int u = 0; u < 4; ++u) {
                    if (!(g0 + 2 * u < ngrp)) continue;
                    const float *q = acc_q + 16 * (g0 + 2 * u);
#pragma unroll
                    for (int wi = 0; wi < 4; ++wi) {
                        const float4 qa = *reinterpret_cast<const float4 *>(q + 4 * wi);
#pragma unroll
                        for (int v = 0; v < 2; ++v) {
                            const uint32_t wv = wi == 0 ? cv[v][u].x : (wi == 1 ? cv[v][u].y : (wi == 2 ? cv[v][u].z : cv[v][u].w));
                            const float e0 = fmaf(par[v].y, (float)(wv & 255u), par[v].x) - qa.x;
                            const float e1 = fmaf(par[v].y, (float)((wv >> 8) & 255u), par[v].x) - qa.y;
                            const float e2 = fmaf(par[v].y, (float)((wv >> 16) & 255u), par[v].x) - qa.z;
                            const float e3 = fmaf(par[v].y, (float)(wv >> 24), par[v].x) - qa.w;
                            d0[v] = fmaf(e0, e0, d0[v]), d1[v] = fmaf(e1, e1, d1[v]), d0[v] = fmaf(e2, e2, d0[v]), d1[v] = fmaf(e3, e3, d1[v]);
                        }
                    }
                    asm volatile("" ::: "memory");
                }
            }
#pragma unroll
            for (int v = 0; v < 2; ++v) {
                float dt = d0[v] + d1[v];
                dt += __shfl_xor(dt, 1, 2);
                const float err = rown ? par[v].w * up : (par[v].z * up) * sqd;
                const float t = sqrtf(dt * down) * down - err * up;
                if (exact[v] && t > 0.0f && (t * t) * (down * down) > thr) {
                    exact[v] = false;
                    if (hf == 0) recs[iv[v]].accurate = __builtin_inff();
                    ++rejected;
                }
            }
        }
#pragma unroll
        for (int v = 0; v < 2; ++v)
            if (exact[v] && hf == 0) queue[atomicAdd(&qn, 1u)] = iv[v];
        __syncthreads();
        uint32_t waiting = qn;
        __syncthreads();
        while (waiting >= 128) {
            const uint32_t j = queue[waiting - 128 + pair];
            const float r = exact_l2_pair(base + (uint64_t)recs[j].pos * dim + 4 * hf, acc_q, dim, hf);
            if (hf == 0) recs[j].accurate = r;
            waiting -= 128;
            __syncthreads();
            if (threadIdx.x == 0) qn = waiting;
            __syncthreads();
        }
    }
    const uint32_t waiting = qn;
    if (pair < waiting) {
        const uint32_t j = queue[pair];
        const float r = exact_l2_pair(base + (uint64_t)recs[j].pos * dim + 4 * hf, acc_q, dim, hf);
        if (hf == 0) recs[j].accurate = r;
    }
    uint32_t rj = hf == 0 ? rejected : 0u;
#pragma unroll
    for (int o = 32; o >= 1; o >>= 1) rj += __shfl_xor(rj, o, 64);
    if ((threadIdx.x & 63) == 0 && rj) atomicAdd(&nshadow[b], rj);
}

__global__ __launch_bounds__(256) void accurate_kernel(SurvRec *__restrict__ surv,
                                                       const unsigned long long *__restrict__ surv_cnt,
                                                       const QSeg seg, const BaseView base,
                                                       const float *__restrict__ qpad, uint32_t dim,
                                                       const uint32_t *__restrict__ order,
                                                       const uint32_t *__restrict__ probe_cluster, uint32_t nprobe) {
    extern __shared__ __attribute__((aligned(16))) float acc_q[];
    const uint32_t b = order ? order[blockIdx.y] : blockIdx.y;
    const uint32_t n = (uint32_t)surv_cnt[b];
    if (n > seg.capof(b) || n == 0) return;
    for (uint32_t c = threadIdx.x * 4; c < dim; c += 1024)
        *reinterpret_cast<float4 *>(acc_q + c) = *reinterpret_cast<const float4 *>(qpad + (uint64_t)b * dim + c);
    __syncthreads();
    accurate_rows(surv + seg.at(b), n, base, acc_q, dim, blockIdx.x * 128 + (threadIdx.x >> 1), gridDim.x * 128,
                  probe_cluster + (uint64_t)b * nprobe);
}

__global__ __launch_bounds__(64) void sort_runs_kernel(RunRec *__restrict__ runs,
                                                        const unsigned long long *__restrict__ surv_cnt,
                                                        const QSeg seg, uint32_t *__restrict__ big_list,
                                                        uint32_t *__restrict__ big_count, uint32_t list_above,
                                                        const RunRec *runs_src) {
    const uint32_t b = blockIdx.x;
    const unsigned long long c = surv_cnt[b];
    if ((uint32_t)c > seg.capof(b)) return;
    const uint32_t nruns = (uint32_t)(c >> 32);
    if (list_above != 512u) {
        if (nruns > list_above && threadIdx.x == 0) big_list[atomicAdd(big_count, 1u)] = b;
        return;
    }
    if (nruns > 512) {
        if (threadIdx.x == 0) big_list[atomicAdd(big_count, 1u)] = b;
        return;
    }
    sort_segment<RunRec, 512>(runs + seg.at(b), nruns, runs_src ? runs_src + seg.at(b) : nullptr);
}

__global__ __launch_bounds__(256) void sort_runs_mid_kernel(RunRec *__restrict__ runs, RunRec *__restrict__ runs_tmp,
                                                            const unsigned long long *__restrict__ surv_cnt, const QSeg seg,
                                                            const uint32_t *__restrict__ big_list,
                                                            uint32_t *__restrict__ big_count ,
                                                            uint32_t nslots, uint32_t src_is_tmp, uint32_t lds_words) {
    extern __shared__ __attribute__((aligned(16))) uint32_t mid_lds[];
    const uint32_t total = big_count[0];
    for (uint32_t i = blockIdx.x; i < total; i += gridDim.x) {
        const uint32_t b = big_list[i], n = (uint32_t)(surv_cnt[b] >> 32);
        RunRec *dir = runs + seg.at(b), *tmp = runs_tmp ? runs_tmp + seg.at(b) : nullptr;
        bool done = false;
        if (nslots <= 1024 && tmp && lds_words) {
            if (src_is_tmp) {
                done = order_runs_bitmap<1024>(tmp, dir, n, nslots, mid_lds, mid_lds + lds_words, lds_words);
// ... 135 lines not shown
                }
            }
#pragma unroll
            for (int v = 0; v < 2; ++v)
                if (dst[v] != ~0ull) surv[dst[v]] = rec[v];
        }
        __builtin_amdgcn_fence(__ATOMIC_SEQ_CST, "wavefront");
    }
}

__global__ __launch_bounds__(1024) void seg_scan_kernel(const uint32_t *__restrict__ q_cap, uint32_t nq,
                                                        unsigned long long *__restrict__ q_base, unsigned long long *__restrict__ out_total) {
    __shared__ unsigned long long wsum[16];
    __shared__ unsigned long long carry;
    const uint32_t tid = threadIdx.x, lane = tid & 63, wid = tid >> 6;
    if (tid == 0) carry = 0;
    __syncthreads();
    for (uint32_t base = 0; base < nq; base += 1024) {
        const uint32_t i = base + tid;
        const unsigned long long v = i < nq ? q_cap[i] : 0ull;
        unsigned long long incl = v;
        for (int o = 1; o < 64; o <<= 1) {
            const unsigned long long up = __shfl_up(incl, o, 64);
            if ((int)lane >= o) incl += up;
        }
        if (lane == 63) wsum[wid] = incl;
        __syncthreads();
        unsigned long long woff = 0;
        for (uint32_t w = 0; w < wid; ++w) woff += wsum[w];
        const unsigned long long c0 = carry;
        if (i < nq) q_base[i] = c0 + woff + incl - v;
        __syncthreads();
        if (tid == 1023) carry = c0 + woff + incl;
        __syncthreads();
    }
    if (tid == 0) out_total[0] = carry;
}

__global__ void clear_dir_kernel(RunRec *__restrict__ runs, uint32_t nq, const QSeg seg, uint32_t ncells) {
    const uint64_t i = (uint64_t)blockIdx.x * blockDim.x + threadIdx.x;
    if (i >= (uint64_t)nq * ncells) return;
    const uint32_t b = (uint32_t)(i / ncells), c = (uint32_t)(i - (uint64_t)b * ncells);
    RunRec z;
    z.pos = 0, z.slot = 0, z.base = 0, z.cnt = 0;
    runs[seg.at(b) + c] = z;
}

__global__ void init_state_kernel(ReplayState st, unsigned long long *__restrict__ surv_cnt, uint32_t nq,
                                  const float *__restrict__ thr_init, const uint32_t *__restrict__ row_map) {
    uint32_t b = blockIdx.x * blockDim.x + threadIdx.x;
    if (b >= nq) return;
    st.thr[b] = thr_init ? thr_init[row_map ? row_map[b] : b] : 3.402823466e+38f;
    st.recent_max[b] = -3.402823466e+38f;
    st.heap_len[b] = 0, st.precise[b] = 0, st.need[b] = 0, st.ovf[b] = 0, st.nsurv[b] = 0, st.nshadow[b] = 0, st.win_count[b] = 0, st.arr_len[b] = 0;
    surv_cnt[b] = 0;
}

__global__ void finalize_heap_kernel(const ReplayState st, uint32_t nq, uint32_t topk,
                                     const uint32_t *__restrict__ row_map, const uint32_t *__restrict__ map_ids,
                                     float *__restrict__ out_dist, uint32_t *__restrict__ out_id,
                                     uint32_t *__restrict__ out_n) {
    uint32_t i = blockIdx.x * blockDim.x + threadIdx.x;
    if (i >= nq * topk) return;
    uint32_t b = i / topk, e = i - b * topk;
    uint32_t ob = row_map ? row_map[b] : b;
    uint32_t len = st.heap_len[b];
    if (e < len) {
        out_dist[(uint64_t)ob * topk + e] = ord32_to_f32(st.heap_key[(uint64_t)b * topk + e]);
        out_id[(uint64_t)ob * topk + e] = map_ids[st.heap_id[(uint64_t)b * topk + e]];
    }
    if (e == 0) out_n[ob] = len;
}

__global__ void finalize_heuristic_kernel(const ReplayState st, uint32_t nq, uint32_t topk,
                                          const uint32_t *__restrict__ row_map, const uint32_t *__restrict__ map_ids,
                                          float *__restrict__ out_dist, uint32_t *__restrict__ out_id,
                                          uint32_t *__restrict__ out_n) {
    uint32_t i = blockIdx.x * blockDim.x + threadIdx.x;
    if (i >= nq * topk) return;
    uint32_t b = i / topk, e = i - b * topk;
    uint32_t ob = row_map ? row_map[b] : b;
    uint32_t len = st.arr_len[b];
    len = len < st.hcap ? len : st.hcap;
    uint32_t take = len < topk ? len : topk;
    if (e < take) {
        const SurvRec &r = st.arr[(uint64_t)b * st.hcap + e];
        out_dist[(uint64_t)ob * topk + e] = r.rough;
        out_id[(uint64_t)ob * topk + e] = map_ids[__builtin_bit_cast(uint32_t, r.accurate)];
    }
    if (e == 0) out_n[ob] = take;
}

__global__ __launch_bounds__(64) void stat_fold_kernel(const unsigned long long *__restrict__ stat, unsigned long long *__restrict__ out) {
    unsigned long long a = stat[2 * threadIdx.x], b = stat[2 * threadIdx.x + 1];
    for (int o = 32; o >= 1; o >>= 1) a += __shfl_xor(a, o, 64), b += __shfl_xor(b, o, 64);
    if (threadIdx.x == 0) out[0] = a, out[1] = b;
}
__global__ __launch_bounds__(256) void metrics_sum_kernel(const unsigned long long *__restrict__ rough,
                                                          const uint32_t *__restrict__ precise,
                                                          const uint32_t *__restrict__ need,
                                                          const uint32_t *__restrict__ arr_len,
                                                          const uint32_t *__restrict__ nsurv,
                                                          const uint32_t *__restrict__ nshadow, uint32_t nq,
                                                          const uint32_t *__restrict__ ovf, uint32_t hcap,
                                                          unsigned long long *__restrict__ out4) {
    __shared__ unsigned long long s[6];
    if (threadIdx.x < 6) s[threadIdx.x] = 0;
    __syncthreads();
    unsigned long long r = 0, p = 0, o = 0, a = 0, mx = 0, sh = 0;
    for (uint32_t i = blockIdx.x * 256 + threadIdx.x; i < nq; i += gridDim.x * 256) {
        const bool ok = !ovf[i] && (!arr_len || arr_len[i] <= hcap);
        r += rough[i];
        p += ok ? precise[i] : 0;
        o += ok ? 0 : 1;
        a += nsurv[i];
        sh += nshadow[i];
        const unsigned long long al = arr_len ? arr_len[i] : 0ull;
        unsigned long long nd = need[i] > al ? (unsigned long long)need[i] : al;
        mx = nd > mx ? nd : mx;
    }
    atomicAdd(&s[0], r);
    atomicAdd(&s[1], p);
    atomicAdd(&s[2], o);
    atomicAdd(&s[3], a);
    atomicMax(&s[4], mx);
    atomicAdd(&s[5], sh);
    __syncthreads();
    if (threadIdx.x < 4) atomicAdd(&out4[threadIdx.x], s[threadIdx.x]);
    if (threadIdx.x == 5) atomicAdd(&out4[5], s[5]);
    if (threadIdx.x == 4) atomicMax(&out4[4], s[4]);
}
```

rabitq_amd/csrc/rabitq_hip.hip:

```cpp
#include "../../include/rabitq_hip.h"

#include <hip/hip_runtime.h>

#include <algorithm>
#include <charconv>
#include <chrono>
#include <atomic>
#include <cmath>
#include <cstdio>
#include <cstdlib>
#include <cstring>
#include <memory>
#include <mutex>
#include <random>
#include <string>
#include <thread>
#include <vector>
#include <sys/stat.h>
#include <dlfcn.h>
#include <queue>
#include <map>

#include "common.h"
#include "kernels_build.h"
// ... 396 lines not shown
                if (good) metric_name.assign(v0, in.p);
            } else good = in.skip();
        } while (good && in.lit(','));
        good = good && in.need('}');
    }
    if (!good) return fail(RQ_ERR_IO, std::string("deserialize error in ") + path + (in.err.empty() ? "" : ": " + in.err));
    uint32_t metric = RQ_METRIC_L2;
    if (metric_name == "\"cosine\"") metric = RQ_METRIC_COSINE;
    else if (!metric_name.empty() && metric_name != "\"l2\"") return fail(RQ_ERR_IO, std::string("unknown metric ") + metric_name + " in " + path);
    const uint64_t n = ids.size(), k = off.empty() ? 0 : off.size() - 1;
    if (dim == 0 || dim % 64 || pr != dim || pc != dim || P.size() != dim * dim || br != dim || bc != n || base.size() != dim * n ||
        cr != dim || cc != k || cent.size() != dim * k || off.empty() || fac.size() != n || codes.size() != n * (dim / 64) ||
        off.back() != n)
        return fail(RQ_ERR_IO, std::string("inconsistent index in ") + path);
    for (uint64_t j = 0; j + 1 < off.size(); ++j)
        if (off[j] > off[j + 1]) return fail(RQ_ERR_IO, "offsets are not non-decreasing");
    std::vector<float> base_rows(n * dim), cent_rows(k * dim);
    for (uint64_t i = 0; i < dim; ++i) {
        for (uint64_t j = 0; j < n; ++j) base_rows[j * dim + i] = base[i * n + j];
        for (uint64_t j = 0; j < k; ++j) cent_rows[j * dim + i] = cent[i * k + j];
    }
    std::vector<uint32_t> off32(off.begin(), off.end()), ids32(ids.begin(), ids.end());
    std::vector<uint64_t> codes64(codes.begin(), codes.end());
    return from_arrays((uint32_t)dim, n, (uint32_t)k, base_rows.data(), P.data(), cent_rows.data(), off32.data(), ids32.data(),
                       codes64.data(), fac.data(), metric, out);
}

void rq_free(rq_index *idx) { delete idx; }

rq_status rq_info(const rq_index *idx, rq_info_t *out) {
    if (!idx || !out) return fail(RQ_ERR_INVALID, "null argument");
    rq_info_t full{};
    full.dim = idx->dim, full.k = idx->k, full.n = idx->n, full.max_list_len = idx->max_list_len, full.n_hbm = idx->n_dev;
    full.split_rows = idx->split_rows ? 1u : 0u, full.metric = idx->metric;
    return copy_out_sized(out, full);
}

rq_status rq_get_device_ptr(const rq_index *idx, int which, const void **out_ptr, uint64_t *out_bytes) {
    if (!idx || !out_ptr || !out_bytes) return fail(RQ_ERR_INVALID, "null argument");
    switch (which) {
        case RQ_ARR_BASE:
            if (idx->n_dev < idx->n)
                return fail(RQ_ERR_UNSUPPORTED, "the raw vectors of this index are tiered (HBM + pinned host memory): no single device array; use rq_get_array");
            if (idx->split_rows)
                return fail(RQ_ERR_UNSUPPORTED, "the raw vectors of this index are stored as split rows (two 16-bit planes per row): no f32 device array; use rq_get_array");
            *out_ptr = idx->base.p, *out_bytes = idx->n_dev * idx->dim * 4;
            break;
        case RQ_ARR_ORTHOGONAL: *out_ptr = idx->P.p, *out_bytes = (uint64_t)idx->dim * idx->dim * 4; break;
        case RQ_ARR_CENTROIDS: *out_ptr = idx->centroids.p, *out_bytes = (uint64_t)idx->k * idx->dim * 4; break;
        case RQ_ARR_OFFSETS: *out_ptr = idx->offsets.p, *out_bytes = ((uint64_t)idx->k + 1) * 4; break;
        case RQ_ARR_MAP_IDS: *out_ptr = idx->map_ids.p, *out_bytes = idx->n * 4; break;
        case RQ_ARR_CODES: *out_ptr = idx->codes.p, *out_bytes = idx->n * idx->W * 8; break;
        case RQ_ARR_FACTORS: *out_ptr = idx->factors.p, *out_bytes = idx->n * 16; break;
        default: return fail(RQ_ERR_INVALID, "unknown array id");
    }
    return RQ_OK;
}

rq_status rq_get_array(const rq_index *idx, int which, void *dst, uint64_t dst_bytes) {
    const void *p;
    uint64_t bytes;
    if (idx && which == RQ_ARR_BASE && (idx->n_dev < idx->n || idx->split_rows)) {
        if (!dst || dst_bytes < idx->n * idx->dim * 4) return fail(RQ_ERR_INVALID, "destination too small");
        return copy_base_rows(idx, 0, idx->n, static_cast<float *>(dst), false);
    }
    RQC(rq_get_device_ptr(idx, which, &p, &bytes));
    if (!dst || dst_bytes < bytes) return fail(RQ_ERR_INVALID, "destination too small");
    if (bytes) HIPC(hipMemcpy(dst, p, bytes, hipMemcpyDeviceToHost));
    return RQ_OK;
}

rq_status rq_coarse_topk_device(const rq_index *idx, const float *d_queries, uint32_t nq, uint32_t len,
                                uint32_t list_lo, uint32_t list_hi, uint32_t probe, uint32_t *d_out_cluster,
                                float *d_out_dist) {
    RQC(ensure_device());
    if (!idx || !d_queries || !d_out_cluster || !d_out_dist) return fail(RQ_ERR_INVALID, "null argument");
    if (idx->dim != (len + 63) / 64 * 64) return fail(RQ_ERR_DIM_MISMATCH, "query length does not pad to dim");
    if (probe == 0 || list_lo >= list_hi || list_hi > idx->k) return fail(RQ_ERR_INVALID, "bad list range / probe");
    if (probe > RQ_MAX_PROBE) return fail(RQ_ERR_UNSUPPORTED, "probe > 16384");
    if (nq == 0) return RQ_OK;
    const uint32_t dim = idx->dim, kc = list_hi - list_lo, np = std::min(probe, kc);
    rq_index *mi = const_cast<rq_index *>(idx);
    Workspace *ws = ws_acquire(mi);
    WsLease rel(mi, ws);
    if (!ws->stream) HIPC(hipStreamCreateWithFlags(&ws->stream, hipStreamNonBlocking));
    hipStream_t st = ws->stream;
    const uint32_t chunk = (uint32_t)std::min<uint64_t>(nq, std::max<uint64_t>(1024, (1ull << 31) / std::max(kc, idx->k)));
    RQC(ws->y.ensure((uint64_t)chunk * dim));
    RQC(ws->dist.ensure((uint64_t)chunk * std::max(kc, idx->k)));
    const bool cosine = idx->metric == RQ_METRIC_COSINE;
    if (len != dim || cosine) RQC(ws->qpad.ensure((uint64_t)chunk * dim));
    for (uint32_t q0 = 0; q0 < nq; q0 += chunk) {
        const uint32_t m = std::min(chunk, nq - q0);
        const float *qp = d_queries + (uint64_t)q0 * len;
        if (cosine) {
            launch_normalize(qp, m, len, dim, ws->qpad.p, st);
            qp = ws->qpad.p;
        } else if (len != dim) {
            pad_rows_kernel<<<ceil_div((uint64_t)m * dim, 256), 256, 0, st>>>(qp, ws->qpad.p, m, len, dim);
            qp = ws->qpad.p;
        }
        launch_rotate(qp, idx->P.p, ws->y.p, m, dim, m >= 32, st);
        if (kc == idx->k && coarse_prefilter_applies(idx, m, np)) {
            RQC(ws->coarse_redo.ensure(m));
            RQC(ws->qf6.ensure((size_t)m * dim / 2 + 16));
            launch_coarse_prefiltered(idx, ws->y.p, ws->dist.p, m, np, d_out_cluster + (uint64_t)q0 * probe, d_out_dist + (uint64_t)q0 * probe, probe, nullptr,
// ... 340 lines not shown
        g_coarse_tiled_from = value;
        return RQ_OK;
    }
    if (std::string(name) == "coarse_impl") {
        if (value < 0 || value > 4) return fail(RQ_ERR_INVALID, "coarse_impl must be 0, 1, 2, 3 or 4");
        g_coarse_impl = value;
        return RQ_OK;
    }
    if (std::string(name) == "survivor_segments") {
#ifdef RQ_DEV_ABLATIONS
        if (value < 0 || value > 3) return fail(RQ_ERR_INVALID, "survivor_segments must be 0, 1, 2 or 3");
#else
        if (value == 3) return fail(RQ_ERR_INVALID, "survivor_segments = 3 (allocation-failure injection) exists in the developer build only (make dev)");
        if (value < 0 || value > 2) return fail(RQ_ERR_INVALID, "survivor_segments must be 0, 1 or 2");
#endif
        g_seg_opt = value;
        return RQ_OK;
    }
    if (std::string(name) == "assign_impl") {
        if (value < 0 || value > 1) return fail(RQ_ERR_INVALID, "assign_impl must be 0 or 1");
        g_assign_impl = value;
        return RQ_OK;
    }
    if (std::string(name) == "small_batch_span") {
        if (value < 1) return fail(RQ_ERR_INVALID, "small_batch_span must be >= 1");
        g_sb_span = value;
        return RQ_OK;
    }
    if (std::string(name) == "small_batch") {
        if (value < 0 || value > 1) return fail(RQ_ERR_INVALID, "small_batch must be 0 or 1");
        g_small_batch = value;
        return RQ_OK;
    }
    if (std::string(name) == "dense_dir") {
        if (value < 0 || value > 1) return fail(RQ_ERR_INVALID, "dense_dir must be 0 or 1");
        g_dense_dir = value;
        return RQ_OK;
    }
    if (std::string(name) == "shared_thresholds") {
        if (value < 0 || value > 2) return fail(RQ_ERR_INVALID, "shared_thresholds must be 0, 1 or 2");
        g_shared_thr = value;
        return RQ_OK;
    }
    if (std::string(name) == "group_rank") {
        if (value < 0 || value > 2) return fail(RQ_ERR_INVALID, "group_rank must be 0, 1 or 2");
        g_group_rank = value;
        return RQ_OK;
    }
    if (std::string(name) == "prep_placement") {
        if (value < 0 || value > 1) return fail(RQ_ERR_INVALID, "prep_placement must be 0 or 1");
        g_prep_placement = value;
        return RQ_OK;
    }
    if (std::string(name) == "rerank_shadow") {
        if (value < 0 || value > 2) return fail(RQ_ERR_INVALID, "rerank_shadow must be 0 (never), 1 (fp16 rows when they fit) or 2 (8-bit rows when they fit)");
        g_rerank_shadow = value;
        return RQ_OK;
    }
    if (std::string(name) == "scan_gate") {
        if (value < 0 || value > 2) return fail(RQ_ERR_INVALID, "scan_gate must be 0, 1 or 2");
        g_scan_gate = value;
        return RQ_OK;
    }
    if (std::string(name) == "scan_debug") {
#ifdef RQ_DEV_ABLATIONS
        const int allowed = 0x7FFFFFFF;
#else
        const int allowed = 128 | 512 | 4096 | 16384;
#endif
        if (value < 0 || (value & ~allowed)) return fail(RQ_ERR_INVALID, "scan_debug: this bit exists in the developer build only (librabitq_hip_dev.so)");
        g_scan_dbg = value;
        return RQ_OK;
    }
    return fail(RQ_ERR_INVALID, std::string("unknown option ") + name);
}

rq_status rq_set_profiling(int level) {
    if (level < 0 || level > 2) return fail(RQ_ERR_INVALID, "profiling level must be 0, 1 or 2");
    g_profiling = level;
    return RQ_OK;
}
rq_status rq_last_profile(rq_profile_t *out) {
    if (!out) return fail(RQ_ERR_INVALID, "null argument");
    return copy_out_sized(out, g_profile);
}

rq_status rq_rotate(const float *x, uint64_t n, uint32_t dim, const float *orthogonal, int use_mfma, float *out) {
    RQC(ensure_device());
    if (!x || !orthogonal || !out) return fail(RQ_ERR_INVALID, "null argument");
    if (dim == 0 || dim % 64) return fail(RQ_ERR_DIM_MISMATCH, "dim must be a multiple of 64");
    DevBuf<float> dx, dp, dout;
    RQC(dx.alloc(n * dim));
    RQC(dp.alloc((size_t)dim * dim));
    RQC(dout.alloc(n * dim));
    HIPC(hipMemcpy(dx.p, x, n * dim * 4, hipMemcpyHostToDevice));
    HIPC(hipMemcpy(dp.p, orthogonal, (size_t)dim * dim * 4, hipMemcpyHostToDevice));
    launch_rotate(dx.p, dp.p, dout.p, n, dim, use_mfma != 0, nullptr);
    HIPC(hipDeviceSynchronize());
    HIPC(hipGetLastError());
    HIPC(hipMemcpy(out, dout.p, n * dim * 4, hipMemcpyDeviceToHost));
    return RQ_OK;
}

rq_status rq_rotate_device(const rq_index *idx, const float *d_x, uint64_t n, float *d_out, float *out_ms) {
    RQC(ensure_device());
    if (!idx || !d_x || !d_out) return fail(RQ_ERR_INVALID, "null argument");
// ... 169 lines not shown
```

rabitq_amd/index.py:

```python
from __future__ import annotations

import ctypes as C
import os

import numpy as np

from . import _lib
from ._lib import BuildStatsT, Info, MetricsT, ProfileT, check, lib

ARR_BASE, ARR_ORTHOGONAL, ARR_CENTROIDS, ARR_OFFSETS, ARR_MAP_IDS, ARR_CODES, ARR_FACTORS = range(7)


def _addr(a):
    return C.c_void_p(a.ctypes.data) if a is not None else C.c_void_p(0)


def _f32(a):
    return np.ascontiguousarray(a, dtype=np.float32)


def pack_filter_bits(ids=None, mask=None, nbits=None):
    if (ids is None) == (mask is None):
        raise ValueError("give exactly one of ids / mask")
    if mask is not None:
        m = np.ascontiguousarray(mask, dtype=bool).reshape(-1)
        nb = m.size
    else:
        a = np.asarray(ids).reshape(-1)
        if a.size and (not np.issubdtype(a.dtype, np.integer) or a.min() < 0):
            raise ValueError("ids must be non-negative integers")
        a = a.astype(np.uint64, copy=False)
        nb = int(a.max()) + 1 if nbits is None and a.size else int(nbits or 0)
        m = np.zeros(nb, dtype=bool)
        m[a[a < nb].astype(np.int64)] = True
    if nbits is not None and mask is not None and int(nbits) != nb:
        raise ValueError("nbits must equal the mask's length")
    if nb > (1 << 32):
        raise ValueError("ids are u32: nbits <= 2^32")
    nwords = (nb + 31) // 32
    packed = np.packbits(m, bitorder="little")
    buf = np.zeros(nwords * 4, dtype=np.uint8)
    buf[:packed.size] = packed
    return buf.view(np.uint32), nb


class Filter:

    def __init__(self, index: "RaBitQ", handle):
        self.index = index
        self._h = handle
        rows = C.c_uint64()
        check(lib().rq_filter_rows(self._h, C.byref(rows)))
        self.rows = int(rows.value)

    def close(self):
        if getattr(self, "_h", None):
            lib().rq_filter_free(self._h)
            self._h = None

    def __enter__(self):
        return self

    def __exit__(self, *exc):
# ... 125 lines not shown
                                          _addr(centroids), _addr(offsets), _addr(map_ids), _addr(codes), _addr(factors),
                                          _lib.metric_id(metric), C.byref(h)))
        return cls(h)

    def rotate_device(self, x_ptr: int, n: int, out_ptr: int) -> float:
        ms = C.c_float()
        check(lib().rq_rotate_device(self._h, C.c_void_p(x_ptr), n, C.c_void_p(out_ptr), C.byref(ms)))
        return float(ms.value)

    def close(self):
        if getattr(self, "_h", None):
            lib().rq_free(self._h)
            self._h = None

    def __del__(self):
        try:
            self.close()
        except Exception:
            pass

    def _get(self, which, shape, dtype):
        out = np.empty(shape, dtype=dtype)
        check(lib().rq_get_array(self._h, which, _addr(out), out.nbytes))
        return out

    @property
    def base(self):
        return self._get(ARR_BASE, (self.n, self.dim), np.float32)

    @property
    def orthogonal(self):
        return self._get(ARR_ORTHOGONAL, (self.dim, self.dim), np.float32)

    @property
    def centroids(self):
        return self._get(ARR_CENTROIDS, (self.k, self.dim), np.float32)

    @property
    def offsets(self):
        return self._get(ARR_OFFSETS, (self.k + 1,), np.uint32)

    @property
    def map_ids(self):
        return self._get(ARR_MAP_IDS, (self.n,), np.uint32)

    @property
    def codes(self):
        return self._get(ARR_CODES, (self.n, self.dim // 64), np.uint64)

    @property
    def factors(self):
        return self._get(ARR_FACTORS, (self.n, 4), np.float32)

    def device_ptr(self, which):
        p, nbytes = C.c_void_p(), C.c_uint64()
        check(lib().rq_get_device_ptr(self._h, which, C.byref(p), C.byref(nbytes)))
        return p.value, nbytes.value

    def make_filter(self, ids=None, mask=None) -> Filter:
        words, nbits = pack_filter_bits(ids=ids, mask=mask)
        h = C.c_void_p()
        check(lib().rq_filter_create(self._h, _addr(words), nbits, 0, C.byref(h)))
        return Filter(self, h)

    def make_filter_device(self, bits_ptr: int, nbits: int) -> Filter:
        h = C.c_void_p()
        check(lib().rq_filter_create(self._h, C.c_void_p(bits_ptr), nbits, 1, C.byref(h)))
        return Filter(self, h)

    def _rows(self, vectors):
        v = np.asarray(vectors)
        if v.dtype.kind not in "fiu":
            raise TypeError(f"vectors must be real numbers, not {v.dtype}")
        if v.ndim != 2:
            raise ValueError(f"vectors must be 2-D (m x d), not {v.ndim}-D")
        if v.shape[1] == 0 or (v.shape[1] + 63) // 64 * 64 != self.dim:
            raise _lib.RabitqError(-2, f"row length {v.shape[1]} does not pad to index dim {self.dim}")
        return _f32(v)

    @staticmethod
    def _ids(ids, m):
        a = np.asarray(ids)
        if a.dtype.kind not in "iu":
            raise TypeError(f"ids must be integers, not {a.dtype}")
        if a.ndim != 1 or a.size != m:
            raise ValueError(f"ids must be 1-D with one id per row ({m}), not shape {a.shape}")
        if a.size and (int(a.min()) < 0 or int(a.max()) > 0xFFFFFFFF):
            raise ValueError("ids are u32: 0 <= id < 2^32")
        return np.ascontiguousarray(a, dtype=np.uint32)

    def add(self, vectors, ids=None) -> np.ndarray:
        rows = self._rows(vectors)
        m = rows.shape[0]
        idv = self._ids(ids, m) if ids is not None else None
        first = C.c_uint32()
        check(lib().rq_add(self._h, _addr(rows), m, rows.shape[1], _addr(idv), 0, C.byref(first)))
        self._refresh()
        return idv.copy() if idv is not None else np.arange(m, dtype=np.uint64).astype(np.uint32) + np.uint32(first.value)

    def add_device(self, rows_ptr: int, m: int, d: int, ids_ptr: int = None) -> int:
        first = C.c_uint32()
        check(lib().rq_add(self._h, C.c_void_p(rows_ptr), m, d, C.c_void_p(ids_ptr or 0), 1, C.byref(first)))
        self._refresh()
        return int(first.value)

    def remove(self, ids=None, mask=None) -> int:
# ... 210 lines not shown
```

Before: 3.950 million.

## Add second 8-bit residual shadow plane to prefilter rerank candidates

Builds a second 8-bit plane that quantizes the residual of the first q8 shadow encoding, using per-list residual ranges. The filtered rerank kernel gets a templated path that uses this plane to tighten the lower-bound distance and reject more candidates before the exact fp32 L2 check. The goal is to cut full-precision base-row reads during rerank. In exchange it adds another n×dim bytes of HBM, extra build kernels, a second queue stage in the rerank kernel, and more LDS per probe.

```diff
diff --git a/include/rabitq_hip.h b/include/rabitq_hip.h
--- a/include/rabitq_hip.h
+++ b/include/rabitq_hip.h
@@ -104,7 +104,8 @@
 
 rq_status rq_info(const rq_index *idx, rq_info_t *out);
 enum { RQ_ARR_BASE = 0, RQ_ARR_ORTHOGONAL, RQ_ARR_CENTROIDS, RQ_ARR_OFFSETS, RQ_ARR_MAP_IDS,
-       RQ_ARR_CODES, RQ_ARR_FACTORS };
+       RQ_ARR_CODES, RQ_ARR_FACTORS,
+       RQ_ARR_SHADOW_Q8, RQ_ARR_SHADOW_Q8_LISTS, RQ_ARR_SHADOW_Q8B, RQ_ARR_SHADOW_Q8B_LISTS };
 rq_status rq_get_array(const rq_index *idx, int which, void *dst, uint64_t dst_bytes);
 rq_status rq_get_device_ptr(const rq_index *idx, int which, const void **out_ptr, uint64_t *out_bytes);
 
@@ -227,6 +228,7 @@
     uint64_t survivor_workspace_bytes;
     uint32_t segmented_passes;
     uint32_t matrix_additive_launches;
+    uint64_t rerank_plane2_rejects;
 } rq_profile_t;
 rq_status rq_set_profiling(int level);
 rq_status rq_set_option(const char *name, int value);
diff --git a/rabitq_amd/_lib.py b/rabitq_amd/_lib.py
--- a/rabitq_amd/_lib.py
+++ b/rabitq_amd/_lib.py
@@ -74,7 +74,8 @@
         ("ms_scan_matrix", C.c_float), ("matrix_launches", C.c_uint32), ("matrix_pairs", C.c_uint64),
         ("matrix_subtile_steps", C.c_uint64), ("matrix_exact_steps", C.c_uint64),
         ("rerank_shadow_rejects", C.c_uint64), ("ms_early", C.c_float), ("small_batch_passes", C.c_uint32),
-        ("survivor_workspace_bytes", C.c_uint64), ("segmented_passes", C.c_uint32), ("matrix_additive_launches", C.c_uint32)]
+        ("survivor_workspace_bytes", C.c_uint64), ("segmented_passes", C.c_uint32), ("matrix_additive_launches", C.c_uint32),
+        ("rerank_plane2_rejects", C.c_uint64)]
 
 
 class MutateStatsT(_Sized):
diff --git a/rabitq_amd/csrc/host_build.h b/rabitq_amd/csrc/host_build.h
--- a/rabitq_amd/csrc/host_build.h
+++ b/rabitq_amd/csrc/host_build.h
@@ -63,6 +63,8 @@
     idx->base_h.release();
     idx->base_q8.release();
     idx->list_q8.release();
+    idx->base_q8b.release();
+    idx->list_q8b.release();
     int kind = g_rerank_shadow.load();
     if (kind == 2 && idx->dim > 4096) kind = 1;
     if (!kind || idx->base_host != nullptr || idx->split_rows || idx->n < RQ_SHADOW_MIN_ROWS) return RQ_OK;
@@ -77,15 +79,33 @@
             idx->list_q8.release();
             return RQ_OK;
         }
+        if (g_shadow_plane2.load() != 0) {
+            HIPC(hipMemGetInfo(&free_b, &total_b));
+            if (!(free_b < bytes + (48ull << 30) && bytes > (1ull << 30)) &&
+                (idx->base_q8b.alloc(total) != RQ_OK || idx->list_q8b.alloc(std::max<uint32_t>(idx->k, 1)) != RQ_OK)) {
+                (void)hipGetLastError();
+                idx->base_q8b.release();
+                idx->list_q8b.release();
+            }
+            if (!idx->list_q8b.p) idx->base_q8b.release();
+        }
+        float4 *const par2 = idx->base_q8b.p ? idx->list_q8b.p : nullptr;
         std::vector<uint32_t> off((size_t)idx->k + 1);
         HIPC(hipMemcpy(off.data(), idx->offsets.p, off.size() * 4, hipMemcpyDeviceToHost));
         uint32_t longest = 0;
         for (uint32_t c = 0; c < idx->k; ++c) longest = std::max(longest, off[c + 1] - off[c]);
-        q8_range_kernel<<<idx->k, 256>>>(idx->base.p, idx->offsets.p, idx->dim, idx->list_q8.p);
+        q8_range_kernel<<<idx->k, 256>>>(idx->base.p, idx->offsets.p, idx->dim, idx->list_q8.p, par2);
         if (longest)
             for (uint32_t c0 = 0; c0 < idx->k; c0 += 32768)
                 q8_encode_kernel<<<dim3(ceil_div(longest, 256u), std::min(32768u, idx->k - c0)), 256>>>(
-                    idx->base.p, idx->offsets.p + c0, idx->dim, idx->list_q8.p + c0, idx->base_q8.p);
+                    idx->base.p, idx->offsets.p + c0, idx->dim, idx->list_q8.p + c0, idx->base_q8.p, par2 ? par2 + c0 : nullptr);
+        if (par2) {
+            q8b_params_kernel<<<ceil_div(std::max<uint32_t>(idx->k, 1), 256u), 256>>>(idx->list_q8.p, par2, idx->k);
+            if (longest)
+                for (uint32_t c0 = 0; c0 < idx->k; c0 += 32768)
+                    q8b_encode_kernel<<<dim3(ceil_div(longest, 256u), std::min(32768u, idx->k - c0)), 256>>>(
+                        idx->base.p, idx->offsets.p + c0, idx->dim, idx->list_q8.p + c0, idx->base_q8.p, par2 + c0, idx->base_q8b.p);
+        }
         HIPC(hipDeviceSynchronize());
         HIPC(hipGetLastError());
         return RQ_OK;
diff --git a/rabitq_amd/csrc/host_mutate.h b/rabitq_amd/csrc/host_mutate.h
--- a/rabitq_amd/csrc/host_mutate.h
+++ b/rabitq_amd/csrc/host_mutate.h
@@ -180,6 +180,7 @@
 
     swap_buf(idx->base, nx->base), swap_buf(idx->P, nx->P), swap_buf(idx->centroids, nx->centroids), swap_buf(idx->cent_t, nx->cent_t);
     swap_buf(idx->base_h, nx->base_h), swap_buf(idx->base_q8, nx->base_q8), swap_buf(idx->list_q8, nx->list_q8);
+    swap_buf(idx->base_q8b, nx->base_q8b), swap_buf(idx->list_q8b, nx->list_q8b);
     swap_buf(idx->offsets, nx->offsets), swap_buf(idx->map_ids, nx->map_ids), swap_buf(idx->codes, nx->codes);
     swap_buf(idx->factors, nx->factors), swap_buf(idx->list_uref, nx->list_uref), swap_buf(idx->cent_bf, nx->cent_bf);
     swap_buf(idx->cent_sqnorm, nx->cent_sqnorm), swap_buf(idx->row_key, nx->row_key);
diff --git a/rabitq_amd/csrc/host_plan.h b/rabitq_amd/csrc/host_plan.h
--- a/rabitq_amd/csrc/host_plan.h
+++ b/rabitq_amd/csrc/host_plan.h
@@ -34,6 +34,7 @@
 
 struct PassPlan {
     uint32_t nprobe, npairs;
+    bool shadow_plane2;
     uint32_t dbg;
     bool small;
     uint32_t sb_nstages, sb_lo[RQ_SB_MAX_STAGES], sb_hi[RQ_SB_MAX_STAGES], sb_final_lo;
@@ -78,6 +79,7 @@
     const uint32_t min_len = filt ? 0u : idx->min_list_len;
     const int impl = g_scan_impl.load();
     pl.dbg = (uint32_t)g_scan_dbg.load();
+    pl.shadow_plane2 = g_shadow_plane2.load() != 0;
     const int gate_opt = g_scan_gate.load(), rank_opt = g_group_rank.load(), tt_opt = g_scan_tile_table.load(), gopt = g_stage_growth.load();
     const bool dense_opt = g_dense_dir.load() != 0, additive_loose = idx->additive_loose.load() != 0;
     const uint64_t settle_pct = (uint64_t)g_stage_settle_pct.load();
diff --git a/rabitq_amd/csrc/host_query.h b/rabitq_amd/csrc/host_query.h
--- a/rabitq_amd/csrc/host_query.h
+++ b/rabitq_amd/csrc/host_query.h
@@ -38,6 +38,7 @@
     RQC(ws.q_base.ensure(nq));
     RQC(ws.nsurv.ensure(nq));
     RQC(ws.nshadow.ensure(nq));
+    RQC(ws.nshadow2.ensure(nq));
     RQC(ws.recent.ensure(nq));
     RQC(ws.win_count.ensure(nq));
     RQC(ws.arr_len.ensure(nq));
@@ -93,6 +94,7 @@
         prof_acc->scan_bytes += res->rough * (uint64_t)(dim / 8 + 16);
         prof_acc->rerank_candidates += ws.h_totals[3];
         prof_acc->rerank_shadow_rejects += ws.h_totals[5];
+        prof_acc->rerank_plane2_rejects += ws.h_totals[6];
         if (g_scan_dbg.load() & 256) {
             unsigned long long ht[12];
             HIPC(hipMemcpy(ht, ws.stat.p + 128, sizeof ht, hipMemcpyDeviceToHost));
@@ -541,10 +543,14 @@
         pf.begin(PF_RERANK);
         const uint32_t gx = std::max(1u, std::min(16u, 4096u / std::max(nq, 1u)));
         const bool prefilter = (r.no > 0 || qp.thr_init) && !(pl.dbg & 512);
-        if (idx->base_q8.p && prefilter)
-            accurate_filtered8_kernel<<<dim3(gx, nq), 256, (size_t)dim * sizeof(float) + (nprobe <= RQ_ACC8_LDS_PROBES ? (size_t)nprobe * 16 : 0), st>>>(
+        if (idx->base_q8.p && prefilter && idx->base_q8b.p && pl.shadow_plane2)
+            accurate_filtered8_kernel<true><<<dim3(gx, nq), 256, (size_t)dim * sizeof(float) + (nprobe <= RQ_ACC8_LDS_PROBES ? (size_t)nprobe * 32 : 0), st>>>(
                 ws.surv.p, ws.surv_cnt.p, seg, idx->base.p, idx->base_q8.p, idx->list_q8.p, qpad, dim, rerank_order, ws.thr.p,
-                probe_cluster, nprobe, ws.nshadow.p, k);
+                probe_cluster, nprobe, ws.nshadow.p, k, idx->base_q8b.p, idx->list_q8b.p, ws.nshadow2.p);
+        else if (idx->base_q8.p && prefilter)
+            accurate_filtered8_kernel<false><<<dim3(gx, nq), 256, (size_t)dim * sizeof(float) + (nprobe <= RQ_ACC8_LDS_PROBES ? (size_t)nprobe * 16 : 0), st>>>(
+                ws.surv.p, ws.surv_cnt.p, seg, idx->base.p, idx->base_q8.p, idx->list_q8.p, qpad, dim, rerank_order, ws.thr.p,
+                probe_cluster, nprobe, ws.nshadow.p, k, nullptr, nullptr, nullptr);
         else if (idx->base_h.p && prefilter)
             accurate_filtered_kernel<<<dim3(gx, nq), 256, (size_t)dim * sizeof(float), st>>>(
                 ws.surv.p, ws.surv_cnt.p, seg, idx->base.p, idx->base_h.p, qpad, dim, rerank_order, ws.thr.p,
@@ -592,7 +598,7 @@
             }
             metrics_sum_kernel<<<std::min(256u, ceil_div(nq, 256)), 256, 0, st>>>(
                 ws.rough_cnt.p, ws.precise.p, ws.need.p, qp.heuristic ? ws.arr_len.p : nullptr, ws.nsurv.p, ws.nshadow.p, nq, ws.ovf.p, qp.hcap,
-                ws.totals.p);
+                ws.totals.p, ws.nshadow2.p);
         }
         pf.end();
         if (pf.on) (void)hipEventRecord(pf.spans[total_span].b, st);
@@ -619,7 +625,7 @@
     Pass c{idx, ws, qp, pl, ws.prof, ws.stream, idx->dim, idx->k, idx->W, qp.nq, qp.topk, pl.nprobe, pl.npairs, d_q, d_row_map, ext_cluster, ext_dist,
            d_out_dist, d_out_id, d_out_n, prof_acc, d_q, ws.probe_cluster.p, ws.probe_dist.p};
     c.rs.thr = ws.thr.p, c.rs.heap_len = ws.heap_len.p, c.rs.heap_key = ws.heap_key.p, c.rs.heap_id = ws.heap_id.p;
-    c.rs.precise = ws.precise.p, c.rs.need = ws.need.p, c.rs.nsurv = ws.nsurv.p, c.rs.nshadow = ws.nshadow.p, c.rs.recent_max = ws.recent.p, c.rs.win_count = ws.win_count.p;
+    c.rs.precise = ws.precise.p, c.rs.need = ws.need.p, c.rs.nsurv = ws.nsurv.p, c.rs.nshadow = ws.nshadow.p, c.rs.nshadow2 = ws.nshadow2.p, c.rs.recent_max = ws.recent.p, c.rs.win_count = ws.win_count.p;
     c.rs.arr_len = ws.arr_len.p, c.rs.arr = ws.arr.p, c.rs.hcap = qp.hcap, c.rs.ovf = ws.ovf.p;
     c.pend.nq = qp.nq, c.pend.cap = qp.cap, c.pend.filter = qp.filter, c.pend.range = qp.range;
     Prof &pf = ws.prof;
diff --git a/rabitq_amd/csrc/host_shard.h b/rabitq_amd/csrc/host_shard.h
--- a/rabitq_amd/csrc/host_shard.h
+++ b/rabitq_amd/csrc/host_shard.h
@@ -113,6 +113,7 @@
     acc.retries += x.retries, acc.ms_scan_matrix += x.ms_scan_matrix, acc.matrix_launches += x.matrix_launches;
     acc.matrix_pairs += x.matrix_pairs, acc.matrix_subtile_steps += x.matrix_subtile_steps;
     acc.matrix_exact_steps += x.matrix_exact_steps, acc.rerank_shadow_rejects += x.rerank_shadow_rejects;
+    acc.rerank_plane2_rejects += x.rerank_plane2_rejects;
     acc.ms_early += x.ms_early, acc.small_batch_passes += x.small_batch_passes;
     acc.survivor_workspace_bytes = std::max(acc.survivor_workspace_bytes, x.survivor_workspace_bytes), acc.segmented_passes += x.segmented_passes;
     acc.matrix_additive_launches += x.matrix_additive_launches;
diff --git a/rabitq_amd/csrc/host_state.h b/rabitq_amd/csrc/host_state.h
--- a/rabitq_amd/csrc/host_state.h
+++ b/rabitq_amd/csrc/host_state.h
@@ -187,7 +187,7 @@
     DevBuf<uint32_t> pair_rank, rank_base;
     DevBuf<uint32_t> img_final, pair_begin, fin_rank, fin_rank_base, fin_grp_cnt, fin_grp_start;
     DevBuf<uint32_t> probe_cluster, recs, grp_cnt, grp_start, heap_len, heap_id, precise, need,
-        nsurv, nshadow, win_count, arr_len, row_map, big_list;
+        nsurv, nshadow, nshadow2, win_count, arr_len, row_map, big_list;
     DevBuf<int32_t> heap_key;
     DevBuf<PairScalars> scal;
     DevBuf<uint64_t> planes;
@@ -244,6 +244,8 @@
     DevBuf<_Float16> base_h;
     DevBuf<uint8_t> base_q8;
     DevBuf<float4> list_q8;
+    DevBuf<uint8_t> base_q8b;
+    DevBuf<float4> list_q8b;
     DevBuf<uint32_t> offsets, map_ids;
     DevBuf<uint64_t> codes;
     DevBuf<float4> factors;
@@ -596,6 +598,7 @@
 static std::atomic<int> g_cluster_major_div{32};
 static std::atomic<int> g_stage_settle_pct{100};
 static std::atomic<int> g_scan_tile_table{1};
+static std::atomic<int> g_shadow_plane2{1};
 static std::atomic<int> g_prep_placement{1};
 static std::atomic<int> g_group_rank{1};
 static std::atomic<int> g_shared_thr{1};
diff --git a/rabitq_amd/csrc/kernels_query.h b/rabitq_amd/csrc/kernels_query.h
--- a/rabitq_amd/csrc/kernels_query.h
+++ b/rabitq_amd/csrc/kernels_query.h
@@ -1910,6 +1910,7 @@
     uint32_t *ovf;
     uint32_t *nsurv;
     uint32_t *nshadow;
+    uint32_t *nshadow2;
     float *recent_max;
     uint32_t *win_count;
     uint32_t *arr_len;
@@ -2462,7 +2463,7 @@
     return tpr >= 1 && tpr <= 64 && (tpr & (tpr - 1)) == 0;
 }
 __global__ __launch_bounds__(256) void q8_range_kernel(const float *__restrict__ base, const uint32_t *__restrict__ offsets, uint32_t dim,
-                                                       float4 *__restrict__ list_q8) {
+                                                       float4 *__restrict__ list_q8, float4 *__restrict__ list_q8b) {
     __shared__ float smn[4], smx[4];
     __shared__ uint32_t sbad[4];
     const uint32_t c = blockIdx.x;
@@ -2494,11 +2495,37 @@
         if (!(sc > 0.0f)) sc = 1.0f;
         if (!(sc < 3.0e38f) || !(fabsf(lo) < 3.0e38f)) bad = 1;
         list_q8[c] = make_float4(bad ? 0.0f : lo, bad ? 1.0f : sc, bad ? __builtin_inff() : 0.0f, bad ? __builtin_inff() : 0.0f);
+        if (list_q8b) list_q8b[c] = make_float4(__builtin_bit_cast(float, 0xFFFFFFFFu), __builtin_bit_cast(float, 0u), 0.0f, 0.0f);
+    }
+}
+__device__ __forceinline__ uint32_t q8_residual_key(float f) {
+    const uint32_t u = __builtin_bit_cast(uint32_t, f);
+    return (u >> 31) ? ~u : (u | 0x80000000u);
+}
+__device__ __forceinline__ float q8_residual_of_key(uint32_t k) {
+    return __builtin_bit_cast(float, (k >> 31) ? (k & 0x7FFFFFFFu) : ~k);
+}
+__device__ __forceinline__ void q8_fold_errors(float emax, float nmax, uint32_t dim, bool row_norms, float4 *rec, float *smax, float *snorm) {
+#pragma unroll
+    for (int o = 32; o >= 1; o >>= 1) {
+        const float a = __shfl_xor(emax, o, 64), b = __shfl_xor(nmax, o, 64);
+        emax = a > emax ? a : emax, nmax = b > nmax ? b : nmax;
+    }
+    if ((threadIdx.x & 63) == 0) smax[threadIdx.x >> 6] = emax, snorm[threadIdx.x >> 6] = nmax;
+    __syncthreads();
+    if (threadIdx.x == 0) {
+        for (int w2 = 1; w2 < 4; ++w2) emax = smax[w2] > emax ? smax[w2] : emax, nmax = snorm[w2] > nmax ? snorm[w2] : nmax;
+        atomicMax(reinterpret_cast<unsigned int *>(&rec->z), __builtin_bit_cast(unsigned int, emax));
+        const float nrm = sqrtf(nmax) * (1.0f + (float)(dim + 8) * 6.0e-8f);
+        if (row_norms) atomicMax(reinterpret_cast<unsigned int *>(&rec->w), __builtin_bit_cast(unsigned int, nrm));
     }
 }
 __global__ __launch_bounds__(256) void q8_encode_kernel(const float *__restrict__ base, const uint32_t *__restrict__ offsets, uint32_t dim,
-                                                        float4 *__restrict__ list_q8, uint8_t *__restrict__ out) {
+                                                        float4 *__restrict__ list_q8, uint8_t *__restrict__ out, float4 *__restrict__ list_q8b) {
     __shared__ float smax[4], snorm[4];
+    __shared__ uint32_t srlo, srhi;
+    if (threadIdx.x == 0) srlo = 0xFFFFFFFFu, srhi = 0u;
+    __syncthreads();
     const uint32_t c = blockIdx.y, r0 = offsets[c] + blockIdx.x * 256u, r1 = offsets[c + 1];
     if (r0 >= r1) return;
     const float4 par = list_q8[c];
@@ -2506,10 +2533,82 @@
     const uint32_t tpr = dim / 16, rows_per_pass = 256 / tpr;
     const uint32_t rr = threadIdx.x / tpr, g = threadIdx.x - rr * tpr;
     const bool row_norms = q8_row_norms(dim);
+    float emax = 0.0f, nmax = 0.0f, rlo = 3.402823466e+38f, rhi = -3.402823466e+38f;
+    for (uint32_t r = r0 + rr; r < r1 && r < r0 + 256u && rr < rows_per_pass; r += rows_per_pass) {
+        float e2 = 0.0f;
+        const float *x = base + (uint64_t)r * dim + 16 * g;
+        uint32_t w[4];
+#pragma unroll
+        for (int u = 0; u < 4; ++u) {
+            const float4 v = *reinterpret_cast<const float4 *>(x + 4 * u);
+            const float ve[4] = {v.x, v.y, v.z, v.w};
+            w[u] = 0;
+#pragma unroll
+            for (int i = 0; i < 4; ++i) {
+                float t = rintf((ve[i] - lo) * inv);
+                t = t < 0.0f ? 0.0f : (t > 255.0f ? 255.0f : t);
+                const uint32_t code = (uint32_t)t;
+                const float res = ve[i] - fmaf(sc, (float)code, lo);
+                const float e = fabsf(res);
+                rlo = res < rlo ? res : rlo, rhi = res > rhi ? res : rhi;
+                emax = (e > emax || !(e < 3.0e38f)) ? (e < 3.0e38f ? e : __builtin_inff()) : emax;
+                e2 = fmaf(e, e, e2);
+                w[u] |= code << (8 * i);
+            }
+        }
+        *reinterpret_cast<uint4 *>(out + (uint64_t)r * dim + 16 * g) = make_uint4(w[0], w[1], w[2], w[3]);
+        if (row_norms) {
+            for (uint32_t o = tpr >> 1; o >= 1; o >>= 1) e2 += __shfl_xor(e2, (int)o, 64);
+            nmax = (e2 > nmax || !(e2 < 3.0e38f)) ? (e2 < 3.0e38f ? e2 : __builtin_inff()) : nmax;
+        }
+    }
+    if (list_q8b) {
+#pragma unroll
+        for (int o = 32; o >= 1; o >>= 1) {
+            const float a = __shfl_xor(rlo, o, 64), b = __shfl_xor(rhi, o, 64);
+            rlo = a < rlo ? a : rlo, rhi = b > rhi ? b : rhi;
+        }
+        if ((threadIdx.x & 63) == 0 && rlo <= rhi) atomicMin(&srlo, q8_residual_key(rlo)), atomicMax(&srhi, q8_residual_key(rhi));
+        __syncthreads();
+        if (threadIdx.x == 0 && srlo <= srhi) {
+            atomicMin(reinterpret_cast<unsigned int *>(&list_q8b[c].x), srlo);
+            atomicMax(reinterpret_cast<unsigned int *>(&list_q8b[c].y), srhi);
+        }
+    }
+    q8_fold_errors(emax, nmax, dim, row_norms, &list_q8[c], smax, snorm);
+}
+__global__ __launch_bounds__(256) void q8b_params_kernel(const float4 *__restrict__ list_q8, float4 *__restrict__ list_q8b, uint32_t k) {
+    const uint32_t c = blockIdx.x * 256 + threadIdx.x;
+    if (c >= k) return;
+    const float4 p1 = list_q8[c], acc = list_q8b[c];
+    const uint32_t klo = __builtin_bit_cast(uint32_t, acc.x), khi = __builtin_bit_cast(uint32_t, acc.y);
+    bool bad = !(p1.z < 3.0e38f) || !(p1.w < 3.0e38f);
+    float lo2 = 0.0f, s2 = 1.0f;
+    if (klo <= khi) {
+        lo2 = q8_residual_of_key(klo);
+        s2 = (q8_residual_of_key(khi) - lo2) * (1.0f / 255.0f);
+    }
+    if (!(s2 > 0.0f)) s2 = 1.0f;
+    if (!(s2 < 3.0e38f) || !(fabsf(lo2) < 3.0e38f)) bad = true;
+    list_q8b[c] = make_float4(bad ? 0.0f : lo2, bad ? 1.0f : s2, bad ? __builtin_inff() : 0.0f, bad ? __builtin_inff() : 0.0f);
+}
+__global__ __launch_bounds__(256) void q8b_encode_kernel(const float *__restrict__ base, const uint32_t *__restrict__ offsets, uint32_t dim,
+                                                         const float4 *__restrict__ list_q8, const uint8_t *__restrict__ codes,
+                                                         float4 *__restrict__ list_q8b, uint8_t *__restrict__ out) {
+    __shared__ float smax[4], snorm[4];
+    const uint32_t c = blockIdx.y, r0 = offsets[c] + blockIdx.x * 256u, r1 = offsets[c + 1];
+    if (r0 >= r1) return;
+    const float4 par = list_q8[c], par2 = list_q8b[c];
+    const float lo = par.x, sc = par.y, lo2 = par2.x, s2 = par2.y, inv2 = 1.0f / s2;
+    const uint32_t tpr = dim / 16, rows_per_pass = 256 / tpr;
+    const uint32_t rr = threadIdx.x / tpr, g = threadIdx.x - rr * tpr;
+    const bool row_norms = q8_row_norms(dim);
     float emax = 0.0f, nmax = 0.0f;
     for (uint32_t r = r0 + rr; r < r1 && r < r0 + 256u && rr < rows_per_pass; r += rows_per_pass) {
         float e2 = 0.0f;
         const float *x = base + (uint64_t)r * dim + 16 * g;
+        const uint4 cw = *reinterpret_cast<const uint4 *>(codes + (uint64_t)r * dim + 16 * g);
+        const uint32_t c1[4] = {cw.x, cw.y, cw.z, cw.w};
         uint32_t w[4];
 #pragma unroll
         for (int u = 0; u < 4; ++u) {
@@ -2518,10 +2617,11 @@
             w[u] = 0;
 #pragma unroll
             for (int i = 0; i < 4; ++i) {
-                float t = rintf((ve[i] - lo) * inv);
+                const float x1 = fmaf(sc, (float)((c1[u] >> (8 * i)) & 255u), lo);
+                float t = rintf(((ve[i] - x1) - lo2) * inv2);
                 t = t < 0.0f ? 0.0f : (t > 255.0f ? 255.0f : t);
                 const uint32_t code = (uint32_t)t;
-                const float e = fabsf(ve[i] - fmaf(sc, (float)code, lo));
+                const float e = fabsf(ve[i] - (fmaf(s2, (float)code, lo2) + x1));
                 emax = (e > emax || !(e < 3.0e38f)) ? (e < 3.0e38f ? e : __builtin_inff()) : emax;
                 e2 = fmaf(e, e, e2);
                 w[u] |= code << (8 * i);
@@ -2533,24 +2633,13 @@
             nmax = (e2 > nmax || !(e2 < 3.0e38f)) ? (e2 < 3.0e38f ? e2 : __builtin_inff()) : nmax;
         }
     }
-#pragma unroll
-    for (int o = 32; o >= 1; o >>= 1) {
-        const float a = __shfl_xor(emax, o, 64), b = __shfl_xor(nmax, o, 64);
-        emax = a > emax ? a : emax, nmax = b > nmax ? b : nmax;
-    }
-    if ((threadIdx.x & 63) == 0) smax[threadIdx.x >> 6] = emax, snorm[threadIdx.x >> 6] = nmax;
-    __syncthreads();
-    if (threadIdx.x == 0) {
-        for (int w2 = 1; w2 < 4; ++w2) emax = smax[w2] > emax ? smax[w2] : emax, nmax = snorm[w2] > nmax ? snorm[w2] : nmax;
-        atomicMax(reinterpret_cast<unsigned int *>(&list_q8[c].z), __builtin_bit_cast(unsigned int, emax));
-        const float nrm = sqrtf(nmax) * (1.0f + (float)(dim + 8) * 6.0e-8f);
-        if (row_norms) atomicMax(reinterpret_cast<unsigned int *>(&list_q8[c].w), __builtin_bit_cast(unsigned int, nrm));
-    }
+    q8_fold_errors(emax, nmax, dim, row_norms, &list_q8b[c], smax, snorm);
 }
 
 #ifndef RQ_ACC8_WAVES
 #define RQ_ACC8_WAVES 4
 #endif
+template <bool P2>
 __global__ __launch_bounds__(256, RQ_ACC8_WAVES) void accurate_filtered8_kernel(SurvRec *__restrict__ surv,
                                                                  const unsigned long long *__restrict__ surv_cnt,
                                                                  const QSeg seg, const float *__restrict__ base,
@@ -2559,10 +2648,15 @@
                                                                  const uint32_t *__restrict__ order,
                                                                  const float *__restrict__ thr_start,
                                                                  const uint32_t *__restrict__ probe_cluster, uint32_t nprobe,
-                                                                 uint32_t *__restrict__ nshadow, uint32_t nlists) {
+                                                                 uint32_t *__restrict__ nshadow, uint32_t nlists,
+                                                                 const uint8_t *__restrict__ base_q8b, const float4 *__restrict__ list_q8b,
+                                                                 uint32_t *__restrict__ nshadow2) {
     extern __shared__ __attribute__((aligned(16))) float acc_q[];
     __shared__ uint32_t queue[512];
     __shared__ uint32_t qn;
+    __shared__ uint2 queue_row[P2 ? 512 : 1];
+    __shared__ uint2 queue_c[P2 ? 256 : 1];
+    __shared__ uint32_t qcn;
     const uint32_t b = order ? order[blockIdx.y] : blockIdx.y;
     const uint32_t n = (uint32_t)surv_cnt[b];
     if (n > seg.capof(b) || n == 0) return;
@@ -2579,7 +2673,11 @@
     if (par_lds)
         for (uint32_t sl = threadIdx.x; sl < nprobe; sl += 256)
             lpar[sl] = pc[sl] < nlists ? list_q8[pc[sl]] : make_float4(0.0f, 1.0f, __builtin_inff(), __builtin_inff());
-    if (threadIdx.x == 0) qn = 0;
+    float4 *lpar2 = lpar + nprobe;
+    if (P2 && par_lds)
+        for (uint32_t sl = threadIdx.x; sl < nprobe; sl += 256)
+            lpar2[sl] = pc[sl] < nlists ? list_q8b[pc[sl]] : make_float4(0.0f, 1.0f, __builtin_inff(), __builtin_inff());
+    if (threadIdx.x == 0) qn = 0, qcn = 0;
     __syncthreads();
     const float thr = thr_start[b];
     const bool test = thr > 1e-30f && thr < 3.0e38f;
@@ -2587,7 +2685,59 @@
     const float sqd = sqrtf((float)dim) * 1.001f;
     const bool rown = q8_row_norms(dim);
     const uint32_t ngrp = dim / 16;
-    uint32_t rejected = 0;
+    uint32_t rejected = 0, rejected2 = 0;
+    auto plane2_entry = [&](uint32_t e) {
+        const uint32_t i = queue[e];
+        const uint2 rw = queue_row[e];
+        bool out = false;
+        if (test) {
+            const float4 p1 = par_lds ? lpar[rw.y] : list_q8[pc[rw.y]], p2 = par_lds ? lpar2[rw.y] : list_q8b[pc[rw.y]];
+            const uint8_t *xa = base_q8 + (uint64_t)rw.x * dim, *xb = base_q8b + (uint64_t)rw.x * dim;
+            float d0 = 0.0f, d1 = 0.0f;
+            for (uint32_t g0 = hf; g0 < ngrp; g0 += 8) {
+                uint4 ca[4], cb[4];
+#pragma unroll
+                for (int u = 0; u < 4; ++u)
+                    if (g0 + 2 * u < ngrp) {
+                        ca[u] = *reinterpret_cast<const uint4 *>(xa + 16 * (g0 + 2 * u));
+                        cb[u] = *reinterpret_cast<const uint4 *>(xb + 16 * (g0 + 2 * u));
+                    }
+#pragma unroll
+                for (int u = 0; u < 4; ++u) {
+                    if (!(g0 + 2 * u < ngrp)) continue;
+                    const float *q = acc_q + 16 * (g0 + 2 * u);
+#pragma unroll
+                    for (int wi = 0; wi < 4; ++wi) {
+                        const float4 qa = *reinterpret_cast<const float4 *>(q + 4 * wi);
+                        const uint32_t wa = wi == 0 ? ca[u].x : (wi == 1 ? ca[u].y : (wi == 2 ? ca[u].z : ca[u].w));
+                        const uint32_t wb = wi == 0 ? cb[u].x : (wi == 1 ? cb[u].y : (wi == 2 ? cb[u].z : cb[u].w));
+                        const float e0 = (fmaf(p2.y, (float)(wb & 255u), p2.x) + fmaf(p1.y, (float)(wa & 255u), p1.x)) - qa.x;
+                        const float e1 = (fmaf(p2.y, (float)((wb >> 8) & 255u), p2.x) + fmaf(p1.y, (float)((wa >> 8) & 255u), p1.x)) - qa.y;
+                        const float e2 = (fmaf(p2.y, (float)((wb >> 16) & 255u), p2.x) + fmaf(p1.y, (float)((wa >> 16) & 255u), p1.x)) - qa.z;
+                        const float e3 = (fmaf(p2.y, (float)(wb >> 24), p2.x) + fmaf(p1.y, (float)(wa >> 24), p1.x)) - qa.w;
+                        d0 = fmaf(e0, e0, d0), d1 = fmaf(e1, e1, d1), d0 = fmaf(e2, e2, d0), d1 = fmaf(e3, e3, d1);
+                    }
+                    asm volatile("" ::: "memory");
+                }
+            }
+            float dt = d0 + d1;
+            dt += __shfl_xor(dt, 1, 2);
+            const float err = rown ? p2.w * up : (p2.z * up) * sqd;
+            const float t = sqrtf(dt * down) * down - err * up;
+            out = t > 0.0f && (t * t) * (down * down) > thr;
+        }
+        if (out) {
+            if (hf == 0) recs[i].accurate = __builtin_inff();
+            ++rejected, ++rejected2;
+        } else if (hf == 0) {
+            queue_c[atomicAdd(&qcn, 1u)] = make_uint2(i, rw.x);
+        }
+    };
+    auto exact_entry = [&](uint32_t e) {
+        const uint2 rc = queue_c[e];
+        const float r = exact_l2_pair(base + (uint64_t)rc.y * dim + 4 * hf, acc_q, dim, hf);
+        if (hf == 0) recs[rc.x].accurate = r;
+    };
     for (uint32_t i0 = i_first; i0 < n; i0 += gridDim.x * 256) {
         uint32_t iv[2] = {i0 + pair, i0 + 128 + pair};
         bool exact[2] = {iv[0] < n, iv[1] < n};
@@ -2647,11 +2797,29 @@
         }
 #pragma unroll
         for (int v = 0; v < 2; ++v)
-            if (exact[v] && hf == 0) queue[atomicAdd(&qn, 1u)] = iv[v];
+            if (exact[v] && hf == 0) {
+                const uint32_t e = atomicAdd(&qn, 1u);
+                queue[e] = iv[v];
+                if (P2) queue_row[e] = make_uint2(cur[v].pos, cur[v].slot);
+            }
         __syncthreads();
         uint32_t waiting = qn;
         __syncthreads();
-        while (waiting >= 128) {
+        while (P2 && waiting >= 128) {
+            plane2_entry(waiting - 128 + pair);
+            waiting -= 128;
+            __syncthreads();
+            const uint32_t wc = qcn;
+            if (threadIdx.x == 0) qn = waiting;
+            __syncthreads();
+            if (wc >= 128) {
+                exact_entry(wc - 128 + pair);
+                __syncthreads();
+                if (threadIdx.x == 0) qcn = wc - 128;
+                __syncthreads();
+            }
+        }
+        while (!P2 && waiting >= 128) {
             const uint32_t j = queue[waiting - 128 + pair];
             const float r = exact_l2_pair(base + (uint64_t)recs[j].pos * dim + 4 * hf, acc_q, dim, hf);
             if (hf == 0) recs[j].accurate = r;
@@ -2662,15 +2830,22 @@
         }
     }
     const uint32_t waiting = qn;
-    if (pair < waiting) {
+    if (P2) {
+        if (pair < waiting) plane2_entry(pair);
+        __syncthreads();
+        const uint32_t wc = qcn;
+        for (uint32_t e0 = 0; e0 < wc; e0 += 128)
+            if (e0 + pair < wc) exact_entry(e0 + pair);
+    } else if (pair < waiting) {
         const uint32_t j = queue[pair];
         const float r = exact_l2_pair(base + (uint64_t)recs[j].pos * dim + 4 * hf, acc_q, dim, hf);
         if (hf == 0) recs[j].accurate = r;
     }
-    uint32_t rj = hf == 0 ? rejected : 0u;
-#pragma unroll
-    for (int o = 32; o >= 1; o >>= 1) rj += __shfl_xor(rj, o, 64);
+    uint32_t rj = hf == 0 ? rejected : 0u, rj2 = hf == 0 ? rejected2 : 0u;
+#pragma unroll
+    for (int o = 32; o >= 1; o >>= 1) rj += __shfl_xor(rj, o, 64), rj2 += __shfl_xor(rj2, o, 64);
     if ((threadIdx.x & 63) == 0 && rj) atomicAdd(&nshadow[b], rj);
+    if (P2 && (threadIdx.x & 63) == 0 && rj2) atomicAdd(&nshadow2[b], rj2);
 }
 
 __global__ __launch_bounds__(256) void accurate_kernel(SurvRec *__restrict__ surv,
@@ -2912,7 +3087,7 @@
     if (b >= nq) return;
     st.thr[b] = thr_init ? thr_init[row_map ? row_map[b] : b] : 3.402823466e+38f;
     st.recent_max[b] = -3.402823466e+38f;
-    st.heap_len[b] = 0, st.precise[b] = 0, st.need[b] = 0, st.ovf[b] = 0, st.nsurv[b] = 0, st.nshadow[b] = 0, st.win_count[b] = 0, st.arr_len[b] = 0;
+    st.heap_len[b] = 0, st.precise[b] = 0, st.need[b] = 0, st.ovf[b] = 0, st.nsurv[b] = 0, st.nshadow[b] = 0, st.nshadow2[b] = 0, st.win_count[b] = 0, st.arr_len[b] = 0;
     surv_cnt[b] = 0;
 }
 
@@ -2963,11 +3138,11 @@
                                                           const uint32_t *__restrict__ nsurv,
                                                           const uint32_t *__restrict__ nshadow, uint32_t nq,
                                                           const uint32_t *__restrict__ ovf, uint32_t hcap,
-                                                          unsigned long long *__restrict__ out4) {
-    __shared__ unsigned long long s[6];
-    if (threadIdx.x < 6) s[threadIdx.x] = 0;
-    __syncthreads();
-    unsigned long long r = 0, p = 0, o = 0, a = 0, mx = 0, sh = 0;
+                                                          unsigned long long *__restrict__ out4, const uint32_t *__restrict__ nshadow2) {
+    __shared__ unsigned long long s[7];
+    if (threadIdx.x < 7) s[threadIdx.x] = 0;
+    __syncthreads();
+    unsigned long long r = 0, p = 0, o = 0, a = 0, mx = 0, sh = 0, sh2 = 0;
     for (uint32_t i = blockIdx.x * 256 + threadIdx.x; i < nq; i += gridDim.x * 256) {
         const bool ok = !ovf[i] && (!arr_len || arr_len[i] <= hcap);
         r += rough[i];
@@ -2975,6 +3150,7 @@
         o += ok ? 0 : 1;
         a += nsurv[i];
         sh += nshadow[i];
+        sh2 += nshadow2[i];
         const unsigned long long al = arr_len ? arr_len[i] : 0ull;
         unsigned long long nd = need[i] > al ? (unsigned long long)need[i] : al;
         mx = nd > mx ? nd : mx;
@@ -2985,8 +3161,9 @@
     atomicAdd(&s[3], a);
     atomicMax(&s[4], mx);
     atomicAdd(&s[5], sh);
+    atomicAdd(&s[6], sh2);
     __syncthreads();
     if (threadIdx.x < 4) atomicAdd(&out4[threadIdx.x], s[threadIdx.x]);
-    if (threadIdx.x == 5) atomicAdd(&out4[5], s[5]);
+    if (threadIdx.x == 5 || threadIdx.x == 6) atomicAdd(&out4[threadIdx.x], s[threadIdx.x]);
     if (threadIdx.x == 4) atomicMax(&out4[4], s[4]);
 }
diff --git a/rabitq_amd/csrc/rabitq_hip.hip b/rabitq_amd/csrc/rabitq_hip.hip
--- a/rabitq_amd/csrc/rabitq_hip.hip
+++ b/rabitq_amd/csrc/rabitq_hip.hip
@@ -472,6 +472,10 @@
         case RQ_ARR_MAP_IDS: *out_ptr = idx->map_ids.p, *out_bytes = idx->n * 4; break;
         case RQ_ARR_CODES: *out_ptr = idx->codes.p, *out_bytes = idx->n * idx->W * 8; break;
         case RQ_ARR_FACTORS: *out_ptr = idx->factors.p, *out_bytes = idx->n * 16; break;
+        case RQ_ARR_SHADOW_Q8: *out_ptr = idx->base_q8.p, *out_bytes = idx->base_q8.p ? idx->n * idx->dim : 0; break;
+        case RQ_ARR_SHADOW_Q8_LISTS: *out_ptr = idx->list_q8.p, *out_bytes = idx->base_q8.p ? (uint64_t)idx->k * 16 : 0; break;
+        case RQ_ARR_SHADOW_Q8B: *out_ptr = idx->base_q8b.p, *out_bytes = idx->base_q8b.p ? idx->n * idx->dim : 0; break;
+        case RQ_ARR_SHADOW_Q8B_LISTS: *out_ptr = idx->list_q8b.p, *out_bytes = idx->base_q8b.p ? (uint64_t)idx->k * 16 : 0; break;
         default: return fail(RQ_ERR_INVALID, "unknown array id");
     }
     return RQ_OK;
@@ -918,6 +922,11 @@
         g_prep_placement = value;
         return RQ_OK;
     }
+    if (std::string(name) == "shadow_plane2") {
+        if (value < 0 || value > 1) return fail(RQ_ERR_INVALID, "shadow_plane2 must be 0 or 1");
+        g_shadow_plane2 = value;
+        return RQ_OK;
+    }
     if (std::string(name) == "rerank_shadow") {
         if (value < 0 || value > 2) return fail(RQ_ERR_INVALID, "rerank_shadow must be 0 (never), 1 (fp16 rows when they fit) or 2 (8-bit rows when they fit)");
         g_rerank_shadow = value;
diff --git a/rabitq_amd/index.py b/rabitq_amd/index.py
--- a/rabitq_amd/index.py
+++ b/rabitq_amd/index.py
@@ -9,6 +9,7 @@
 from ._lib import BuildStatsT, Info, MetricsT, ProfileT, check, lib
 
 ARR_BASE, ARR_ORTHOGONAL, ARR_CENTROIDS, ARR_OFFSETS, ARR_MAP_IDS, ARR_CODES, ARR_FACTORS = range(7)
+ARR_SHADOW_Q8, ARR_SHADOW_Q8_LISTS, ARR_SHADOW_Q8B, ARR_SHADOW_Q8B_LISTS = range(7, 11)
 
 
 def _addr(a):
@@ -240,6 +241,15 @@
     def factors(self):
         return self._get(ARR_FACTORS, (self.n, 4), np.float32)
 
+    def shadow_arrays(self):
+        out = []
+        for which, width, dtype in ((ARR_SHADOW_Q8, self.dim, np.uint8), (ARR_SHADOW_Q8_LISTS, 4, np.uint32),
+                                    (ARR_SHADOW_Q8B, self.dim, np.uint8), (ARR_SHADOW_Q8B_LISTS, 4, np.uint32)):
+            _, nbytes = self.device_ptr(which)
+            rows = nbytes // (width * np.dtype(dtype).itemsize)
+            out.append(self._get(which, (rows, width), dtype))
+        return out
+
     def device_ptr(self, which):
         p, nbytes = C.c_void_p(), C.c_uint64()
         check(lib().rq_get_device_ptr(self._h, which, C.byref(p), C.byref(nbytes)))
```

After: 3.874 million. 0.981x the previous value.
